# balbasty/torch-interpol

Measured on AMD Instinct MI355X. Metric: Mvox/s grid_pull & grid_push, 256^3 fp32 cubic/dct2, higher is better.
Workload: dtype f32

## Files before the change

### include/interpol_hip.h

```cpp
#ifndef INTERPOL_HIP_H
#define INTERPOL_HIP_H

#include <stdint.h>

#ifdef __cplusplus
extern "C" {
#endif

#define INTERPOL_ABI_VERSION 1

enum {
    INTERPOL_F32  = 0,
    INTERPOL_F64  = 1,
    INTERPOL_BF16 = 2,
    INTERPOL_F16  = 3
};

enum {
    INTERPOL_OK          =  0,
    INTERPOL_E_DIM       = -1,
    INTERPOL_E_ORDER     = -2,
    INTERPOL_E_BOUND     = -3,
    INTERPOL_E_DTYPE     = -4,
    INTERPOL_E_SHAPE     = -5,
    INTERPOL_E_NULL      = -6,
    INTERPOL_E_EXTRAP    = -7,
    INTERPOL_E_PREFILTER = -8,
    INTERPOL_E_SCRATCH   = -9,
    INTERPOL_E_STRIDE    = -10,
    INTERPOL_E_LAUNCH    = -11
};

typedef struct interpol_problem {
    int32_t abi_version;
    int32_t dim;
    int32_t dtype;
    int32_t grid_dtype;
    int32_t extrapolate;
    int32_t bound[3];
    int32_t order[3];
    int32_t flags;
    int64_t batch;
    int64_t channels;
    int64_t vol_shape[3];
    int64_t grid_shape[3];
    int64_t vol_stride[5];
    int64_t grid_stride[5];
    int64_t val_stride[7];
} interpol_problem;

#define INTERPOL_FLAG_NO_FASTPATH   1
#define INTERPOL_FLAG_ACCUMULATE    2
#define INTERPOL_FLAG_FORCE_TILED   4
#define INTERPOL_FLAG_SEPARABLE_GRID 8
#define INTERPOL_FLAG_DISPLACEMENT  16
#define INTERPOL_FLAG_WITH_COUNT    32
#define INTERPOL_FLAG_BINNED_SCATTER 64
#define INTERPOL_FLAG_AUTO_SCATTER  (1 << 24)
#define INTERPOL_FLAG_SMALL_TILES (1 << 25)
#define INTERPOL_FLAG_SERIAL_ITEMS (1 << 26)
#define INTERPOL_FLAG_GENERAL_KERNELS (1 << 27)
#define INTERPOL_FLAG_SHELL_RUNS (1 << 28)
#define INTERPOL_FLAG_AFFINE_GRID   128

int64_t interpol_scatter_workspace(const interpol_problem *p, int32_t count_only);
int interpol_pull(const interpol_problem *p, const void *vol, const void *grid, void *val, void *stream);
int64_t interpol_pull_workspace(const interpol_problem *p);
int interpol_pull_ws(const interpol_problem *p, const void *vol, const void *grid, void *val, void *workspace, int64_t workspace_bytes, void *stream);
int interpol_grad_ws(const interpol_problem *p, const void *vol, const void *grid, void *val, void *workspace, int64_t workspace_bytes, void *stream);
int interpol_push(const interpol_problem *p, const void *val, const void *grid, void *vol,
                  void *scratch, int64_t scratch_bytes, void *stream);
int interpol_count(const interpol_problem *p, const void *grid, void *vol,
                   void *scratch, int64_t scratch_bytes, void *stream);
int interpol_grad(const interpol_problem *p, const void *vol, const void *grid, void *val, void *stream);
int interpol_pushgrad(const interpol_problem *p, const void *val, const void *grid, void *vol,
                      void *scratch, int64_t scratch_bytes, void *stream);
int interpol_hess(const interpol_problem *p, const void *vol, const void *grid, void *val, void *stream);

int interpol_pull_backward(const interpol_problem *p, const void *grad_out, const void *vol, const void *grid,
                           void *grad_vol, void *grad_grid, void *scratch, int64_t scratch_bytes, void *stream);
int interpol_push_backward(const interpol_problem *p, const void *grad_vol_out, const void *val, const void *grid,
                           void *grad_val, void *grad_grid, void *stream);
int interpol_count_backward(const interpol_problem *p, const void *grad_vol_out, const void *grid,
                            void *grad_grid, void *stream);
int interpol_push_backward_ws(const interpol_problem *p, const void *grad_vol_out, const void *val, const void *grid,
                              void *grad_val, void *grad_grid, void *workspace, int64_t workspace_bytes, void *stream);

int64_t interpol_affine_backward_workspace(const interpol_problem *p);
int interpol_pull_backward_affine(const interpol_problem *p, const void *grad_out, const void *vol,
                                  const void *mat, void *grad_mat,
                                  void *workspace, int64_t workspace_bytes, void *stream);
int interpol_push_backward_affine(const interpol_problem *p, const void *grad_vol_out,
                                  const void *val , const void *mat, void *grad_mat,
                                  void *workspace, int64_t workspace_bytes, void *stream);

int interpol_compose(const interpol_problem *p, const void *left, const void *right, void *out, void *stream);
int interpol_compose_backward_right(const interpol_problem *p, const void *grad_out, const void *left, const void *right,
                                    void *grad_right, void *stream);

int interpol_jacobian(const interpol_problem *p, const void *disp, void *out, int det_only, int add_identity, void *stream);
int interpol_jacdet_backward_field(const interpol_problem *p, const void *grad_out, const void *disp, void *gfield, void *stream);

int interpol_regulariser(const interpol_problem *p, const void *field, void *out, double absolute, double membrane, double bending,
                         const double *voxel_size, void *stream);
int64_t interpol_regulariser_energy_workspace(const interpol_problem *p);
int interpol_regulariser_energy(const interpol_problem *p, const void *field, void *energy, double absolute, double membrane,
                                double bending, const double *voxel_size, void *workspace, int64_t workspace_bytes, void *stream);

int64_t interpol_regulariser_solve_workspace(const interpol_problem *p, int hessian_components);
int interpol_regulariser_solve(const interpol_problem *p, const void *gradient, const void *hessian, int hessian_components,
                               int64_t hessian_batch_stride, void *solution, double absolute, double membrane, double bending,
                               const double *voxel_size, int max_iter, double tolerance, void *info ,
                               void *workspace, int64_t workspace_bytes, void *stream);

int64_t interpol_ssd_workspace(const interpol_problem *p);
int interpol_ssd(const interpol_problem *p, const void *moving, const void *fixed, const void *disp, const void *weight ,
                 void *loss, void *gradient, void *hessian, int hessian_kind, int64_t weight_batch_stride,
                 int64_t gradient_batch_stride, int64_t hessian_batch_stride, void *workspace, int64_t workspace_bytes, void *stream);

int64_t interpol_ssd_affine_workspace(const interpol_problem *p);
int interpol_ssd_affine(const interpol_problem *p, const void *moving, const void *fixed, const void *mat, const void *weight ,
                        void *loss, void *gradient, void *hessian, int with_hessian, int64_t mat_batch_stride,
                        int64_t weight_batch_stride, void *workspace, int64_t workspace_bytes, void *stream);

int64_t interpol_mi_affine_workspace(const interpol_problem *p, int bins);
int interpol_mi_affine(const interpol_problem *p, const void *moving, const void *fixed, const void *mat, const void *weight ,
                       const void *ranges, void *loss, void *gradient, void *hessian, void *histogram , int with_hessian,
                       int bins, int64_t mat_batch_stride, int64_t weight_batch_stride, void *workspace, int64_t workspace_bytes,
                       void *stream);

int64_t interpol_lcc_workspace(const interpol_problem *p);
int interpol_lcc(const interpol_problem *p, const void *moving, const void *fixed, const void *disp, const void *weight ,
                 void *loss, void *gradient, void *hessian, int hessian_kind, const int *window, double eps,
                 int64_t weight_batch_stride, int64_t gradient_batch_stride, int64_t hessian_batch_stride, void *workspace,
                 int64_t workspace_bytes, void *stream);

int64_t interpol_push_bricks_workspace(const interpol_problem *p);
int interpol_push_bricks(const interpol_problem *p, const void *val, const void *grid, void *vol,
                         void *workspace, int64_t workspace_bytes, void *stream);

int interpol_pull_labels(const interpol_problem *p, const void *vol, const void *grid, void *val, void *stream);

int interpol_resample_1d(int32_t dtype, int32_t lin_dtype, int32_t order, int32_t bound, int32_t extrapolate, int32_t mode,
                         int32_t adjoint, int64_t outer, int64_t n_samples, int64_t n_lattice, int64_t inner,
                         const void *src, const void *lin, void *dst, void *stream);
int32_t interpol_resample_1d_gathers(int32_t dtype, int64_t n_samples, int64_t inner);

int interpol_spline_filter(void *data, int32_t dtype, int64_t outer, int64_t n, int64_t inner,
                           int32_t bound, int32_t order, void *stream);
int interpol_spline_filter_to(const void *src, void *data, int32_t dtype, int64_t outer, int64_t n, int64_t inner,
                              int32_t bound, int32_t order, void *stream);

int32_t interpol_host_bound_index(int32_t bound, int32_t i, int32_t n);
int32_t interpol_host_bound_sign(int32_t bound, int32_t i, int32_t n);
double  interpol_host_weight(int32_t order, double x, int32_t which);
float   interpol_host_weight_f32(int32_t order, float x, int32_t which);

#define INTERPOL_HANDBACK_ADAPTIVE 0
#define INTERPOL_HANDBACK_ALWAYS   1
#define INTERPOL_HANDBACK_NEVER    2
int32_t interpol_set_handback(int32_t mode);
int32_t interpol_release_stream(void *stream);

int32_t     interpol_abi_version(void);
int32_t     interpol_has_experiments(void);
const char *interpol_error_string(int code);
const char *interpol_kernel_name(const interpol_problem *p, const char *op);

#ifdef __cplusplus
}
#endif
#endif
```

### torch-interpol_amd/csrc/push_owner.hip

```cpp
#include "sorted_util.hpp"
#include "route.hpp"

namespace ip {
namespace owner {

using namespace sorted;

constexpr int BR = 16;
constexpr int OFF = 160;
constexpr int BOX = BR + 3;
constexpr int PZ = BOX;
constexpr int PLANE = BOX * PZ;
constexpr int BOXSLOTS = BOX * PLANE;
constexpr int NCELL = BR * BR * BR;
constexpr int CAPD = 128;
constexpr int CAPX = 512;
constexpr int NT = 512;
constexpr int NS = TS * TS * TS;
constexpr int NT1 = 512, VPT1 = NS / NT1;
constexpr int LB = 6, NBIN = LB * LB * LB;
constexpr int HDR_SHELL = 34;
constexpr int THIN_SHELL_RUN = 16;
constexpr int KMIX = 13;
template <int K> constexpr int KSV = K == KMIX ? 3 : K;
template <int K> __device__ __forceinline__ int kd(const KParams &p, int d) { return K == KMIX ? p.order[d] : K; }
#ifdef IP_OWNER_MIX_TU
#define IP_KS KSV<K>
#define IP_KD(d) kd<K>(p, d)
#define IP_WX(i) own_weight_x<K>(p, tx, i)
#define IP_MU magic_units_p<K>(p)
#else
#define IP_KS K
#define IP_KD(d) K
#define IP_WX(i) weight_x<K>(tx, i)
#define IP_MU magic_units<K>()
#endif

constexpr int NLO = OFF / BR, NHI = (OFF + 3 + BR - 1) / BR;
struct BrickGrid {
    int nb[3];
    int lo[3], top[3], nin[3], split[3];
    int per_item;
    int item;
    int capd;
};
__host__ __device__ __forceinline__ bool folds(int bound, int n) { return (bound == B_REPLICATE || bound == B_DCT1 || bound == B_DCT2) && n >= 2 * BR; }
static BrickGrid brick_grid(const KParams &k)
{
    BrickGrid g;
    const bool mixed = k.order[0] != k.order[1] || k.order[0] != k.order[2];
    for (int d = 0; d < 3; ++d) {
        const int K = mixed ? 3 : k.order[d], n = k.vol_n[d];
        const bool f = folds(k.bound[d], n);
        g.lo[d] = f ? -(BOX - 1) / 2 : 0;
        g.top[d] = f ? n - (BOX + 1) / 2 + BR : (n - K > 0 ? n - K : 0);
        g.nin[d] = (g.top[d] - g.lo[d] + BR - 1) / BR;
        if (f) {
            const int c = g.top[d] - g.lo[d] - BR * (g.nin[d] - 1);
            if (c < K) { g.top[d] -= c; g.nin[d] -= 1; }
        }
        g.split[d] = f ? g.nin[d] / 2 : (g.nin[d] > 0 ? g.nin[d] - 1 : 0);
        g.nb[d] = NLO + g.nin[d] + NHI;
    }
    g.per_item = g.nb[0] * g.nb[1] * g.nb[2];
    g.item = g.per_item; g.capd = 128;
    return g;
}
__host__ __device__ __forceinline__ int brick_and_cell(int ft, int lo, int top, int nin, int split)
{
    if (ft < lo) return ((ft - lo + OFF) >> 4) | (((ft - lo + OFF) & (BR - 1)) << 16);
    if (ft >= top) return (NLO + nin + ((ft - top) >> 4)) | (((ft - top) & (BR - 1)) << 16);
    const int u = ft - lo, v = top - 1 - ft;
    const bool hi = u >= BR * split && (v >> 4) < nin - 1 - split;
    return hi ? (NLO + nin - 1 - (v >> 4)) | ((BR - 1 - (v & (BR - 1))) << 16) : (NLO + (u >> 4)) | ((u & (BR - 1)) << 16);
}
__host__ __device__ __forceinline__ int brick_origin(int bk, int lo, int top, int nin, int split)
{
    if (bk < NLO) return lo + bk * BR - OFF;
    if (bk >= NLO + nin) return top + (bk - NLO - nin) * BR;
    const int j = bk - NLO;
    return j <= split ? lo + j * BR : top - (nin - j) * BR;
}

__device__ __forceinline__ bool shell_brick(const KParams &p, const BrickGrid &bg, int b0, int b1, int b2)
{
    const int bc[3] = { b0, b1, b2 };
    bool shell = false;
#pragma unroll
    for (int d = 0; d < 3; ++d) shell = shell || bc[d] < NLO + (p.bound[d] == B_DST1 ? 1 : 0) || bc[d] >= NLO + bg.nin[d];
    return shell;
}

struct BinSmem {
    int lo[3], total;
    int cnt[NBIN];
    int base[NBIN];
    int bmx[2];
    int orph, pad_;
    int gbk[NBIN];
};

template <typename T>
__device__ __forceinline__ float src_value(const KParams &p, const T *__restrict__ val, int64_t b, int64_t o, int ch, float m)
{
    if (val == nullptr || ch >= p.C) return m;
    return m * Cvt<float, T>::ld(val[b * p.val_sb + ch * p.val_sc + o]);
}

template <typename T, int K, int GM>
__device__ __forceinline__ void scatter_direct(const KParams &p, const T *__restrict__ val, const float *__restrict__ grid, float *__restrict__ vol,
                                            int64_t b, TileGeom g, int tid, unsigned mask, int nch)
{
    Lattice L;
#pragma unroll
    for (int d = 0; d < 3; ++d) { L.bound[d] = p.bound[d]; L.n[d] = p.vol_n[d]; L.ss[d] = p.vol_ss[d] / 4; L.k[d] = kd<K>(p, d); }
    L.lin = 0;
#pragma unroll 1
    for (int v = 0; v < VPT1; ++v) {
        if (!((mask >> v) & 1)) continue;
        int ox, oy, oz; float x[3];
        sample_pos(g, tid + NT1 * v, ox, oy, oz);
        load_xyz<GM>(p, grid, b, g, ox, oy, oz, x);
        const int64_t o = ((int64_t)ox * g.gy + oy) * g.gz + oz;
        const float m = inb_mask(p, x);
        if (KSV<K> == 1 && p.mode == MODE_ISO0) {
            const long long pk0 = wrap_outofline(L.bound[0], __float2int_rn(rintf(x[0])), L.n[0]);
            const long long pk1 = wrap_outofline(L.bound[1], __float2int_rn(rintf(x[1])), L.n[1]);
            const long long pk2 = wrap_outofline(L.bound[2], __float2int_rn(rintf(x[2])), L.n[2]);
            const float sgn = (float)((int)(pk0 >> 32) * (int)(pk1 >> 32) * (int)(pk2 >> 32));
            float *q = vol + b * p.vol_sb + (int)(pk0 & 0xffffffffll) * L.ss[0] + (int)(pk1 & 0xffffffffll) * L.ss[1] + (int)(pk2 & 0xffffffffll) * L.ss[2];
#pragma unroll 1
            for (int ch = 0; ch < nch; ++ch)
                __hip_atomic_fetch_add(q + (int64_t)ch * p.vol_sc, src_value<T>(p, val, b, o, ch, m) * sgn, __ATOMIC_RELAXED, __HIP_MEMORY_SCOPE_AGENT);
            continue;
        }
        int ii[3]; float tt[3];
#pragma unroll
        for (int d = 0; d < 3; ++d) split(kd<K>(p, d), x[d], ii[d], tt[d]);
#pragma unroll 1
        for (int ch = 0; ch < nch; ++ch)
            tiled::scatter_one_thread(L, vol + b * p.vol_sb + ch * p.vol_sc, src_value<T>(p, val, b, o, ch, m), ii[0], ii[1], ii[2], tt[0], tt[1], tt[2]);
    }
}

template <typename T, int K, int GM>
__device__ __forceinline__ void scatter_orphans(const KParams &p, const T *__restrict__ val, const float *__restrict__ grid, float *__restrict__ vol,
                                             int64_t b, TileGeom g, int tid, unsigned mask, int nch)
{
    Lattice L;
#pragma unroll
    for (int d = 0; d < 3; ++d) { L.bound[d] = p.bound[d]; L.n[d] = p.vol_n[d]; L.ss[d] = p.vol_ss[d] / 4; L.k[d] = kd<K>(p, d); }
    L.lin = 0;
#pragma unroll 1
    for (int v = 0; v < VPT1; ++v) {
        unsigned long long todo = __ballot((mask >> v) & 1);
#pragma unroll 1
        while (todo) {
            const int lane = __ffsll((long long)todo) - 1;
            todo &= todo - 1;
            int ox, oy, oz; float x[3];
            sample_pos(g, (tid & ~63) + lane + NT1 * v, ox, oy, oz);
            load_xyz<GM>(p, grid, b, g, ox, oy, oz, x);
            const int64_t o = ((int64_t)ox * g.gy + oy) * g.gz + oz;
            const float m = inb_mask(p, x);
            if (KSV<K> == 1 && p.mode == MODE_ISO0) { x[0] = rintf(x[0]); x[1] = rintf(x[1]); x[2] = rintf(x[2]); }
            int off;
            const float w = tiled::tap_weight_t<-1, -1>(L, x[0], x[1], x[2], tid & 63, &off, nullptr);
            float *q = vol + b * p.vol_sb + off;
#pragma unroll 1
            for (int ch = 0; ch < nch && w != 0.f; ++ch)
                __hip_atomic_fetch_add(q + (int64_t)ch * p.vol_sc, src_value<T>(p, val, b, o, ch, m) * w, __ATOMIC_RELAXED, __HIP_MEMORY_SCOPE_AGENT);
        }
    }
}

template <typename T, int K, int GM>
__device__ __forceinline__ void gather_direct(const KParams &p, const T *__restrict__ img, const float *__restrict__ grid, T *__restrict__ out,
                                              int64_t b, TileGeom g, int tid, unsigned mask)
{
    Lattice L;
#pragma unroll
    for (int d = 0; d < 3; ++d) { L.bound[d] = p.bound[d]; L.n[d] = p.vol_n[d]; L.ss[d] = p.vol_ss[d] / (int)sizeof(T); L.k[d] = kd<K>(p, d); }
    L.lin = 0;
#pragma unroll 1
    for (int v = 0; v < VPT1; ++v) {
        if (!((mask >> v) & 1)) continue;
        int ox, oy, oz; float x[3];
        sample_pos(g, tid + NT1 * v, ox, oy, oz);
        load_xyz<GM>(p, grid, b, g, ox, oy, oz, x);
        const int64_t o = ((int64_t)ox * g.gy + oy) * g.gz + oz;
        const float m = inb_mask(p, x);
        int ii[3]; float tt[3];
#pragma unroll
        for (int d = 0; d < 3; ++d) split(kd<K>(p, d), x[d], ii[d], tt[d]);
#pragma unroll 1
        for (int ch = 0; ch < p.C; ++ch)
            out[b * p.val_sb + ch * p.val_sc + o] = Cvt<float, T>::st(m * tiled::gather_one_thread<T>(L, img + b * p.vol_sb + ch * p.vol_sc, ii[0], ii[1], ii[2], tt[0], tt[1], tt[2], -1));
    }
}

template <typename T, int K, int GM>
__device__ __forceinline__ void gradc_direct(const KParams &p, const T *__restrict__ img, const T *__restrict__ gout, const float *__restrict__ grid,
                                             float *__restrict__ ggrid, int64_t b, TileGeom g, int tid, unsigned mask)
{
    Lattice L;
#pragma unroll
    for (int d = 0; d < 3; ++d) { L.bound[d] = p.bound[d]; L.n[d] = p.vol_n[d]; L.ss[d] = p.vol_ss[d] / (int)sizeof(T); L.k[d] = kd<K>(p, d); }
    L.lin = 0;
#pragma unroll 1
    for (int v = 0; v < VPT1; ++v) {
        if (!((mask >> v) & 1)) continue;
        int ox, oy, oz; float x[3];
        sample_pos(g, tid + NT1 * v, ox, oy, oz);
        load_xyz<GM>(p, grid, b, g, ox, oy, oz, x);
        const int64_t o = ((int64_t)ox * g.gy + oy) * g.gz + oz;
        const float m = inb_mask(p, x);
        int ii[3]; float tt[3];
#pragma unroll
        for (int d = 0; d < 3; ++d) split(kd<K>(p, d), x[d], ii[d], tt[d]);
        float a[3] = { 0.f, 0.f, 0.f };
#pragma unroll 1
        for (int ch = 0; ch < p.C; ++ch) {
            const float gv = gout ? Cvt<float, T>::ld(gout[b * p.val_sb + ch * p.val_sc + o]) : 1.f;
#pragma unroll 1
            for (int d = 0; d < 3; ++d)
                a[d] = __builtin_fmaf(gv, tiled::gather_one_thread<T>(L, img + b * p.vol_sb + ch * p.vol_sc, ii[0], ii[1], ii[2], tt[0], tt[1], tt[2], d), a[d]);
        }
        float *dst = ggrid + (b * p.N + o) * 3;
        dst[0] = a[0] * m; dst[1] = a[1] * m; dst[2] = a[2] * m;
    }
}

template <typename T, int K, int GM>
__device__ __forceinline__ void grad_direct(const KParams &p, const T *__restrict__ img, const float *__restrict__ grid, T *__restrict__ out,
                                            int64_t b, TileGeom g, int tid, unsigned mask)
{
    Lattice L;
#pragma unroll
    for (int d = 0; d < 3; ++d) { L.bound[d] = p.bound[d]; L.n[d] = p.vol_n[d]; L.ss[d] = p.vol_ss[d] / (int)sizeof(T); L.k[d] = kd<K>(p, d); }
    L.lin = 0;
#pragma unroll 1
    for (int v = 0; v < VPT1; ++v) {
        if (!((mask >> v) & 1)) continue;
        int ox, oy, oz; float x[3];
        sample_pos(g, tid + NT1 * v, ox, oy, oz);
        load_xyz<GM>(p, grid, b, g, ox, oy, oz, x);
        const int64_t o = ((int64_t)ox * g.gy + oy) * g.gz + oz;
        const float m = inb_mask(p, x);
        int ii[3]; float tt[3];
#pragma unroll
        for (int d = 0; d < 3; ++d) split(kd<K>(p, d), x[d], ii[d], tt[d]);
#pragma unroll 1
        for (int ch = 0; ch < p.C; ++ch)
#pragma unroll 1
            for (int d = 0; d < 3; ++d)
                out[b * p.val_sb + ch * p.val_sc + 3 * o + d] =
                    Cvt<float, T>::st(m * tiled::gather_one_thread<T>(L, img + b * p.vol_sb + ch * p.vol_sc, ii[0], ii[1], ii[2], tt[0], tt[1], tt[2], d));
    }
}

template <typename T, int K, int GM, int IDX = 0>
__global__ __launch_bounds__(NT1, 4) void own_bin(KParams p, BrickGrid bg, const T *__restrict__ val, const float *__restrict__ grid,
                                               float *__restrict__ vol, int *__restrict__ ndesc, uint2 *__restrict__ desc,
                                               float4 *__restrict__ rec, float *__restrict__ vals, unsigned short *__restrict__ meta,
                                               int *__restrict__ bmax, int64_t nrec,
                                               int gx, int gy, int gz, int nty, int ntz, int ntiles, const int *__restrict__ gate,
                                               const T *__restrict__ aux, const int *__restrict__ all, int blk0, int thin)
{
    const int blk = (int)blockIdx.x + blk0;
    if (IDX) { const bool every = all && *all == 1; if (gate ? (gate[blk] == 0 && !every) : (all && !every)) return; }
    else if (gate && *gate != 1) return;
    extern __shared__ __attribute__((aligned(16))) unsigned char smem_raw[];
    BinSmem &sm = *reinterpret_cast<BinSmem *>(smem_raw);
    const int tid = threadIdx.x;
    const int64_t b = blk / ntiles;
    const TileGeom g = tile_geom(blk % ntiles, gx, gy, gz, nty, ntz);
    const int nch = (IDX || val == nullptr) ? 1 : p.C + p.cc;
    for (int i = tid; i < NBIN; i += NT1) { sm.cnt[i] = 0; sm.gbk[i] = -1; }
    if (tid < 2) sm.bmx[tid] = 0;
    if (tid == 2) sm.orph = 0;
    if (tid < 3) sm.lo[tid] = 0x7fffffff;
    float c[VPT1][3], v0[VPT1], v1[VPT1];
    unsigned valid = 0;
    prof_mark(-1);
    const bool has0 = !IDX && val != nullptr && p.C > 0, has1 = !IDX && val != nullptr && p.C > 1;
    const T *vp0 = has0 ? val + b * p.val_sb : reinterpret_cast<const T *>(grid);
    const T *vp1 = has1 ? val + b * p.val_sb + p.val_sc : reinterpret_cast<const T *>(grid);
#pragma unroll
    for (int v = 0; v < VPT1; ++v) {
        int ox, oy, oz;
        sample_pos(g, tid + NT1 * v, ox, oy, oz);
        if (ox < gx && oy < gy && oz < gz) valid |= 1u << v;
        ox = ox < gx ? ox : gx - 1; oy = oy < gy ? oy : gy - 1; oz = oz < gz ? oz : gz - 1;
        load_xyz<GM>(p, grid, b, g, ox, oy, oz, c[v]);
        const int64_t o = ((int64_t)ox * gy + oy) * gz + oz;
        if (IDX) { v0[v] = __int_as_float((int)o); v1[v] = 0.f; continue; }
        v0[v] = Cvt<float, T>::ld(vp0[has0 ? o : 0]);
        v1[v] = Cvt<float, T>::ld(vp1[has1 ? o : 0]);
    }
    unsigned inbits = 0;
#pragma unroll
    for (int v = 0; v < VPT1 && !IDX; ++v) {
        const float m = inb_mask(p, c[v]);
        v0[v] = has0 ? v0[v] * m : m; v1[v] = has1 ? v1[v] * m : m;
        if (KSV<K> == 1 && m != 0.f) inbits |= 1u << v;
    }
    if (KSV<K> == 1 && !IDX && p.mode == MODE_ISO0) {
#pragma unroll
        for (int v = 0; v < VPT1; ++v) { c[v][0] = rintf(c[v][0]); c[v][1] = rintf(c[v][1]); c[v][2] = rintf(c[v][2]); }
    }
    int bx[VPT1][3];
    unsigned ok = 0;
    int mn[3] = { 0x7fffffff, 0x7fffffff, 0x7fffffff };
#pragma unroll
    for (int v = 0; v < VPT1; ++v) {
        bool in = (valid >> v) & 1;
#pragma unroll
        for (int d = 0; d < 3; ++d) {
            const float fl = floorf(c[v][d] - 0.5f * (float)(kd<K>(p, d) - 1));
            in = in && fl >= (float)(bg.lo[d] - OFF) && fl < (float)(bg.top[d] + NHI * BR);
            bx[v][d] = in ? brick_and_cell(__float2int_rz(fl), bg.lo[d], bg.top[d], bg.nin[d], bg.split[d]) : 0;
        }
        if (in) {
            ok |= 1u << v;
#pragma unroll
            for (int d = 0; d < 3; ++d) mn[d] = (bx[v][d] & 0xffff) < mn[d] ? (bx[v][d] & 0xffff) : mn[d];
        }
    }
    __syncthreads();
    prof_mark(0);
#pragma unroll
    for (int d = 0; d < 3; ++d) {
        const int a = wave_min(mn[d]);
        if ((tid & 63) == 0) atomicMin(&sm.lo[d], a);
    }
    __syncthreads();
    const int lo[3] = { sm.lo[0], sm.lo[1], sm.lo[2] };
    int lbin[VPT1];
    unsigned local = 0;
#pragma unroll
    for (int v = 0; v < VPT1; ++v) {
        const int r0 = (bx[v][0] & 0xffff) - lo[0], r1 = (bx[v][1] & 0xffff) - lo[1], r2 = (bx[v][2] & 0xffff) - lo[2];
        const bool l = ((ok >> v) & 1) && (unsigned)r0 < (unsigned)LB && (unsigned)r1 < (unsigned)LB && (unsigned)r2 < (unsigned)LB;
        lbin[v] = l ? ((r0 * LB + r1) * LB + r2) | ((bx[v][0] >> 16) << 16 | (bx[v][1] >> 16) << 12 | (bx[v][2] >> 16) << 8) : 0;
        if (l) { local |= 1u << v; lbin[v] |= atomicAdd(&sm.cnt[lbin[v] & 255], 1) << 20; }
    }
    __syncthreads();
    prof_mark(1);
    const int64_t tilebase = (int64_t)blk * NS;
    constexpr int PER = (NBIN + 63) / 64;
    int slot[PER];
    if (tid < 64) {
        int cn[PER], s = 0;
#pragma unroll
        for (int i = 0; i < PER; ++i) { const int e = tid * PER + i; cn[i] = e < NBIN ? sm.cnt[e] : 0; s += cn[i]; }
        int incl = s;
#pragma unroll
        for (int o = 1; o < 64; o <<= 1) { const int t = __shfl_up(incl, o); if (tid >= o) incl += t; }
        int run = incl - s;
        if (tid == 63) sm.total = incl;
        unsigned shl = 0;
        int nsh = 0;
        if (!IDX && thin != 0) {
#pragma unroll
            for (int i = 0; i < PER; ++i) {
                const int e = tid * PER + i;
                if (e < NBIN && cn[i] > 0 && shell_brick(p, bg, lo[0] + e / (LB * LB), lo[1] + (e / LB) % LB, lo[2] + e % LB)) { shl |= 1u << i; nsh += cn[i]; }
            }
#pragma unroll
            for (int o = 32; o > 0; o >>= 1) nsh += __shfl_xor(nsh, o);
        }
        const int lim = thin < 0 ? -thin : thin;
#pragma unroll
        for (int i = 0; i < PER; ++i) {
            const int e = tid * PER + i;
            const int r0 = e / (LB * LB), r1 = (e / LB) % LB, r2 = e % LB;
            const int bk = (int)b * bg.item + ((lo[0] + r0) * bg.nb[1] + (lo[1] + r1)) * bg.nb[2] + (lo[2] + r2);
            slot[i] = 0;
            if (e < NBIN) sm.base[e] = run;
            if (e < NBIN && cn[i] > 0) slot[i] = (((shl >> i) & 1) && (thin > 0 ? nsh : cn[i]) <= lim) ? 0x7fffffff : atomicAdd(&ndesc[bk], 1);
            run += cn[i];
        }
    }
    __syncthreads();
    prof_mark(2);
    int pos[VPT1];
#pragma unroll
    for (int v = 0; v < VPT1; ++v)
        pos[v] = ((local >> v) & 1) ? (sm.base[lbin[v] & 255] + (int)((unsigned)lbin[v] >> 20)) | (((lbin[v] >> 8) & 0xfff) << 16) : -1;
    const bool two = nch > 1;
    int amx0 = 0, amx1 = 0;
#pragma unroll
    for (int v = 0; v < VPT1; ++v) {
        if (pos[v] < 0) continue;
        const int64_t at = tilebase + (pos[v] & 0xffff);
        rec[at] = make_float4(c[v][0], c[v][1], c[v][2], v0[v]);
        if (IDX) continue;
        meta[at] = (unsigned short)(pos[v] >> 16);
        const int a0 = __float_as_int(__builtin_fabsf(v0[v]));
        amx0 = a0 > amx0 ? a0 : amx0;
        if (two) {
            vals[at] = v1[v];
            const int a1 = __float_as_int(__builtin_fabsf(v1[v]));
            amx1 = a1 > amx1 ? a1 : amx1;
        }
    }
    for (int ch = 2; ch < nch && !IDX; ++ch) {
#pragma unroll
        for (int v = 0; v < VPT1; ++v) {
            if (pos[v] < 0) continue;
            int ox, oy, oz;
            sample_pos(g, tid + NT1 * v, ox, oy, oz);
            vals[(int64_t)(ch - 1) * nrec + tilebase + (pos[v] & 0xffff)] = src_value<T>(p, val, b, ((int64_t)ox * gy + oy) * gz + oz, ch, KSV<K> == 1 ? (float)((inbits >> v) & 1u) : inb_mask(p, c[v]));
        }
    }
    if (tid < 64) {
#pragma unroll
        for (int i = 0; i < PER; ++i) {
            const int e = tid * PER + i;
            const int cn = e < NBIN ? sm.cnt[e] : 0;
            if (cn <= 0) continue;
            const int r0 = e / (LB * LB), r1 = (e / LB) % LB, r2 = e % LB;
            const int bk = (int)b * bg.item + ((lo[0] + r0) * bg.nb[1] + (lo[1] + r1)) * bg.nb[2] + (lo[2] + r2);
            if (slot[i] < bg.capd) {
                desc[(int64_t)bk * bg.capd + slot[i]] = make_uint2((unsigned)(tilebase + sm.base[e]), (unsigned)cn);
                sm.gbk[e] = bk;
                if (!IDX && shell_brick(p, bg, lo[0] + r0, lo[1] + r1, lo[2] + r2)) ndesc[HDR_SHELL - 64] = 1;
                if (IDX && slot[i] == 0) bmax[1 + atomicAdd(&bmax[0], 1)] = bk;
            } else { sm.cnt[e] = -1; sm.orph = 1; }
        }
    }
    if (!IDX) {
        amx0 = wave_max(amx0); amx1 = wave_max(amx1);
        if ((tid & 63) == 0) { if (amx0) atomicMax(&sm.bmx[0], amx0); if (amx1) atomicMax(&sm.bmx[1], amx1); }
    }
    __syncthreads();
    for (int e = tid; e < NBIN && !IDX; e += NT1) {
        const int bk = sm.gbk[e];
        if (bk < 0) continue;
        if (sm.bmx[0]) atomicMax(&bmax[2 * (int64_t)bk], sm.bmx[0]);
        if (sm.bmx[1]) atomicMax(&bmax[2 * (int64_t)bk + 1], sm.bmx[1]);
    }
    unsigned direct = valid & ~local;
    if (sm.orph) {
        unsigned orphan = 0;
#pragma unroll
        for (int v = 0; v < VPT1; ++v)
            if (((local >> v) & 1) && sm.cnt[lbin[v] & 255] < 0) orphan |= 1u << v;
        if (IDX) direct |= orphan;
        else scatter_orphans<T, K, GM>(p, val, grid, vol, b, g, tid, orphan, nch);
    }
    if (IDX == 3) { if (direct) grad_direct<T, K, GM>(p, val, grid, reinterpret_cast<T *>(vol), b, g, tid, direct); return; }
    if (IDX == 2) { if (direct) gradc_direct<T, K, GM>(p, val, aux, grid, vol, b, g, tid, direct); return; }
    if (IDX) { if (direct) gather_direct<T, K, GM>(p, val, grid, reinterpret_cast<T *>(vol), b, g, tid, direct); return; }
    if (direct) scatter_direct<T, K, GM>(p, val, grid, vol, b, g, tid, direct, nch);
}

constexpr int VPT = 12;
constexpr int NPIECE = VPT * (NT / 64);
constexpr int BATCH = NPIECE * 64;
constexpr int NCLS = 16;
constexpr int NHW = NT / NCLS;
constexpr unsigned PMASK = 0x1ffffffu;
static_assert(NPIECE <= 128, "a queue entry is piece << 6 | lane in 16 bits");

struct AccSmem {
    int   taboff[3][BOX + 1];
    float tabsgn[3][BOX + 1];
    unsigned ppref[CAPX];
    unsigned start[CAPX];
    uint2 piece[NPIECE];
    int   cmax[2];
    int   dmax, n, npieces;
    int   rlo[3], rhi[3];
    int   qcnt[NCLS];
    int   qsur[NCLS + 1], qhol[NCLS + 1];
    int   qeff[NCLS], qcap;
    union alignas(16) {
        struct {
            unsigned cells[NCELL / 2];
            unsigned short queue[BATCH];
        };
        unsigned nreg[BOX * BOX * (BOX + 1) / 2];
    };
    unsigned long long box[BOXSLOTS];
};
constexpr int NZ = BOX + 1;
static_assert(sizeof(AccSmem) <= 80 * 1024, "two workgroups per CU");
static_assert(sizeof(unsigned) * (BOX * BOX * NZ / 2) <= sizeof(unsigned) * (NCELL / 2) + sizeof(unsigned short) * BATCH, "the stencil counts fit in cells + queue");

constexpr float MAGIC = 12582912.f;
constexpr unsigned MAGIC_ODD = 301u;
template <int K> __device__ __forceinline__ float magic_units() { return K == 3 ? 4194304.f * 0.999f * 3.375f : (K == 2 ? 4194304.f * 0.999f * (64.f / 27.f) : 4194304.f * 0.999f); }
template <int K> __device__ __forceinline__ float magic_cbmax() { return 2147483648.f * 0.99f / magic_units<K>(); }
template <int K> __device__ __forceinline__ float magic_units_p(const KParams &p)
{
    if (K != KMIX) return magic_units<K>();
    float u = 4194304.f * 0.999f;
#pragma unroll
    for (int d = 0; d < 3; ++d) u *= p.order[d] == 3 ? 1.5f : (p.order[d] == 2 ? 4.f / 3.f : 1.f);
    return u;
}

__device__ __forceinline__ void magic_decode(unsigned long long W, unsigned n, int &s0, int &s1)
{
    const unsigned pr = n * MAGIC_ODD;
    const unsigned mlo = pr << 22, mhi = pr >> 10;
    s0 = (int)((unsigned)W - mlo);
    const unsigned long long L = (((unsigned long long)mhi << 32) | mlo) + (unsigned long long)(long long)s0;
    s1 = (int)((unsigned)(W >> 32) - mlo - (unsigned)(L >> 32));
}

template <int I, int J, int NZT = 4>
__device__ __forceinline__ void row_adds(unsigned addr, unsigned long long v0, unsigned long long v1, unsigned long long v2, unsigned long long v3)
{
    constexpr int o = (I * PLANE + J * PZ) * 8;
    if (NZT == 4)
        asm volatile("ds_add_u64 %0, %1 offset:%5\n\tds_add_u64 %0, %2 offset:%6\n\tds_add_u64 %0, %3 offset:%7\n\tds_add_u64 %0, %4 offset:%8"
                     :: "v"(addr), "v"(v0), "v"(v1), "v"(v2), "v"(v3), "n"(o), "n"(o + 8), "n"(o + 16), "n"(o + 24) : "memory");
    else if (NZT == 3)
        asm volatile("ds_add_u64 %0, %1 offset:%4\n\tds_add_u64 %0, %2 offset:%5\n\tds_add_u64 %0, %3 offset:%6"
                     :: "v"(addr), "v"(v0), "v"(v1), "v"(v2), "n"(o), "n"(o + 8), "n"(o + 16) : "memory");
    else
        asm volatile("ds_add_u64 %0, %1 offset:%3\n\tds_add_u64 %0, %2 offset:%4"
                     :: "v"(addr), "v"(v0), "v"(v1), "n"(o), "n"(o + 8) : "memory");
}
template <int K, int I, int J, bool WIDE>
__device__ __forceinline__ void scatter_row(unsigned addr, f2 sx, const f2 *w, int dbg)
{
    const f2 sy = sx * f2{ w[J].x, w[J].x };
    unsigned long long v[4];
#pragma unroll
    for (int k = 0; k < 4; ++k) {
        if (WIDE) {
            v[k] = (unsigned long long)(long long)tiled::cvt_rpi(sy.x * w[k].y);
        } else {
            const f2 pr = __builtin_elementwise_fma(sy, f2{ w[k].y, w[k].y }, f2{ MAGIC, MAGIC });
            v[k] = __builtin_bit_cast(unsigned long long, pr);
        }
    }
#ifdef IP_ABLATE
    if (dbg & 4) { asm volatile("" :: "v"(v[0]), "v"(v[1]), "v"(v[2]), "v"(v[3])); return; }
#endif
    row_adds<I, J, WIDE ? 4 : IP_KS + 1>(addr, v[0], v[1], v[2], v[3]);
}
template <int K, int I, bool WIDE>
__device__ __forceinline__ void scatter_plane(unsigned addr, f2 s, float wxi, const f2 *w, int dbg)
{
#ifdef IP_ABLATE
    if (dbg & 16) {
        const unsigned long long c = 0x100000001ull;
        row_adds<I, 0>(addr, c, c, c, c); row_adds<I, 1>(addr, c, c, c, c); row_adds<I, 2>(addr, c, c, c, c);
        if (IP_KS == 3) row_adds<I, 3>(addr, c, c, c, c);
        return;
    }
#endif
    const f2 sx = s * f2{ wxi, wxi };
    scatter_row<K, I, 0, WIDE>(addr, sx, w, dbg); scatter_row<K, I, 1, WIDE>(addr, sx, w, dbg);
    if (IP_KS >= 2) scatter_row<K, I, 2, WIDE>(addr, sx, w, dbg);
    if (IP_KS == 3) scatter_row<K, I, 3, WIDE>(addr, sx, w, dbg);
}

typedef unsigned short us2 __attribute__((ext_vector_type(2)));
template <int W>
__device__ __forceinline__ void slide(const unsigned *in, unsigned *out)
{
    us2 s = { 0, 0 };
#pragma unroll
    for (int j = 0; j < BOX; ++j) {
        if (j < BR) s += __builtin_bit_cast(us2, in[j]);
        if (j >= W && j - W < BR) s -= __builtin_bit_cast(us2, in[j - W]);
        out[j] = __builtin_bit_cast(unsigned, s);
    }
}
template <int K, typename SM>
__device__ __forceinline__ void stencil_counts(SM &sm, int tid)
{
    constexpr int W = IP_KS + 1, HZ = NZ / 2;
    unsigned *rg = sm.nreg;
    unsigned in[BR], out[BOX];
    if (tid < BR * BR) {
        const uint4 lo = reinterpret_cast<const uint4 *>(sm.cells)[2 * tid], hi = reinterpret_cast<const uint4 *>(sm.cells)[2 * tid + 1];
        in[0] = lo.x; in[1] = lo.y; in[2] = lo.z; in[3] = lo.w; in[4] = hi.x; in[5] = hi.y; in[6] = hi.z; in[7] = hi.w;
    }
    __syncthreads();
    if (tid < BR * BR) {
        int v[BR], o[NZ], s = 0;
#pragma unroll
        for (int i = 0; i < BR / 2; ++i) { v[2 * i] = (int)(in[i] & 0xffffu); v[2 * i + 1] = (int)(in[i] >> 16); }
#pragma unroll
        for (int j = 0; j < BOX; ++j) { if (j < BR) s += v[j]; if (j >= W && j - W < BR) s -= v[j - W]; o[j] = s; }
        o[BOX] = 0;
#pragma unroll
        for (int i = 0; i < HZ; ++i) rg[tid * HZ + i] = (unsigned)o[2 * i] | ((unsigned)o[2 * i + 1] << 16);
    }
    __syncthreads();
    {
        const int x = tid / HZ, zp = tid - x * HZ;
        if (tid < BR * HZ) {
#pragma unroll
            for (int k = 0; k < BR; ++k) in[k] = rg[(x * BR + k) * HZ + zp];
        }
        __syncthreads();
        if (tid < BR * HZ) {
            slide<W>(in, out);
#pragma unroll
            for (int j = 0; j < BOX; ++j) rg[(x * BOX + j) * HZ + zp] = out[j];
        }
        __syncthreads();
    }
    {
        const int y = tid / HZ, zp = tid - y * HZ;
        if (tid < BOX * HZ) {
#pragma unroll
            for (int k = 0; k < BR; ++k) in[k] = rg[(k * BOX + y) * HZ + zp];
        }
        __syncthreads();
        if (tid < BOX * HZ) {
            slide<W>(in, out);
#pragma unroll
            for (int j = 0; j < BOX; ++j) rg[(j * BOX + y) * HZ + zp] = out[j];
        }
        __syncthreads();
    }
}
__device__ __forceinline__ unsigned stencils_at(const AccSmem &sm, int xr, int yr, int zr)
{
    return (unsigned)reinterpret_cast<const unsigned short *>(sm.nreg)[(xr * BOX + yr) * NZ + zr];
}

template <int K> __device__ __forceinline__ float own_weight_x(const KParams &p, float t, int i)
{
    if constexpr (K == KMIX) return mixed_weight_x(p.order[0], t, i);
    else return weight_x<K>(t, i);
}
template <int K> __device__ __forceinline__ float own_wgrad_x(const KParams &p, float t, int i)
{
    if constexpr (K == KMIX) return mixed_wgrad_x(p.order[0], t, i);
    else return wgrad_x<K>(t, i);
}
#ifdef IP_OWNER_MIX_TU
#define IP_RECORD_CELL(...) record_cell<K>(p, __VA_ARGS__)
template <int K>
__device__ __forceinline__ void record_cell(const KParams &p, const float4 &r, const int *b0, int &x0, int &y0, int &z0, float &tx, float &ty, float &tz)
{
    const float fx = floorf(r.x - 0.5f * (float)(kd<K>(p, 0) - 1)), fy = floorf(r.y - 0.5f * (float)(kd<K>(p, 1) - 1)), fz = floorf(r.z - 0.5f * (float)(kd<K>(p, 2) - 1));
#else
#define IP_RECORD_CELL(...) record_cell<K>(__VA_ARGS__)
template <int K>
__device__ __forceinline__ void record_cell(const float4 &r, const int *b0, int &x0, int &y0, int &z0, float &tx, float &ty, float &tz)
{
    const float fx = floorf(r.x - 0.5f * (float)(K - 1)), fy = floorf(r.y - 0.5f * (float)(K - 1)), fz = floorf(r.z - 0.5f * (float)(K - 1));
#endif
    tx = r.x - fx; ty = r.y - fy; tz = r.z - fz;
    x0 = (__float2int_rz(fx) - b0[0]) & (BR - 1); y0 = (__float2int_rz(fy) - b0[1]) & (BR - 1); z0 = (__float2int_rz(fz) - b0[2]) & (BR - 1);
}

__host__ __device__ __forceinline__ int color_first(int color, int d)
{
    if (color >= 8) return 0;
    const int par = (color >> (2 - d)) & 1;
    return NLO + ((par - NLO) & 1);
}
__host__ __device__ __forceinline__ int color_count(int color, int d, const BrickGrid &bg)
{
    if (color >= 8) return bg.nb[d];
    const int j0 = color_first(color, d) - NLO;
    return bg.nin[d] > j0 ? (bg.nin[d] - j0 + 1) >> 1 : 0;
}

template <int K, typename SM>
__device__ __forceinline__ void float_records(const Lattice &L, const SM &sm, float *vc0, float *vc1, bool two, const float4 *__restrict__ rec,
                                              const float *__restrict__ va, const float *__restrict__ vb, const int *b0, int ebeg, int eend)
{
#pragma unroll 1
    for (int e = ebeg; e < eend; e += NHW) {
        const unsigned qe = sm.queue[e];
        const unsigned ri = sm.piece[qe >> 6].x + (qe & 63u);
        const float4 cur = rec[ri];
        const float cs[2] = { va ? va[ri] : cur.w, vb ? vb[ri] : 0.f };
        int x0, y0, z0; float tx, ty, tz;
        record_cell<K>(cur, b0, x0, y0, z0, tx, ty, tz);
#pragma unroll 1
        for (int i = 0; i <= K; ++i) {
            const int gx = b0[0] + x0 + i;
            const int offx = wrap_index(L.bound[0], gx, L.n[0]) * L.ss[0];
            const float fx = tiled::weight1(0, K, tx, i), gsx = (float)wrap_sign(L.bound[0], gx, L.n[0]);
            const float sx0 = cs[0] * fx * gsx, sx1 = cs[1] * fx * gsx;
#pragma unroll 1
            for (int j = 0; j <= K; ++j) {
                const int gy = b0[1] + y0 + j;
                const int offy = wrap_index(L.bound[1], gy, L.n[1]) * L.ss[1];
                const float fy = tiled::weight1(0, K, ty, j), gsy = (float)wrap_sign(L.bound[1], gy, L.n[1]);
                const float sy0 = sx0 * fy * gsy, sy1 = sx1 * fy * gsy;
#pragma unroll 1
                for (int k = 0; k <= K; ++k) {
                    const int gz = b0[2] + z0 + k;
                    const int off = offx + offy + wrap_index(L.bound[2], gz, L.n[2]) * L.ss[2];
                    const float fz = tiled::weight1(0, K, tz, k), gsz = (float)wrap_sign(L.bound[2], gz, L.n[2]);
                    __hip_atomic_fetch_add(vc0 + off, sy0 * fz * gsz, __ATOMIC_RELAXED, __HIP_MEMORY_SCOPE_AGENT);
                    if (two) __hip_atomic_fetch_add(vc1 + off, sy1 * fz * gsz, __ATOMIC_RELAXED, __HIP_MEMORY_SCOPE_AGENT);
                }
            }
        }
    }
}

template <int K, bool NEAR = false, bool SHELL = true>
__global__ __launch_bounds__(NT, 4) void own_accumulate(KParams p, BrickGrid bg, const int *__restrict__ ndesc, const uint2 *__restrict__ desc,
                                                        const float4 *__restrict__ rec, const float *__restrict__ vals,
                                                        const unsigned short *__restrict__ meta, const int *__restrict__ bmax, int64_t nrec,
                                                        float *__restrict__ vol, int nch, int color, int nbatch, const int *__restrict__ gate,
                                                        int *__restrict__ ctr, int bfirst, const int *__restrict__ shell)
{
    if (gate && *gate != 1) return;
    static_assert(SHELL || (K != KMIX && !NEAR), "the colour instantiation: isotropic orders 1 - 3");
    if (SHELL) { if (color == 8 && *shell == 0) return; }
    else __builtin_assume(color >= 0 && color < 8);
    extern __shared__ __attribute__((aligned(16))) unsigned char smem_raw[];
    AccSmem &sm = *reinterpret_cast<AccSmem *>(smem_raw);
    Lattice L;
#pragma unroll
    for (int d = 0; d < 3; ++d) { L.bound[d] = p.bound[d]; L.n[d] = p.vol_n[d]; L.ss[d] = p.vol_ss[d] / 4; L.k[d] = IP_KD(d); }
    L.lin = 0;
    const int step = !SHELL || color < 8 ? 2 : 1;
    const int c0[3] = { color_first(color, 0), color_first(color, 1), color_first(color, 2) };
    const int m0 = color_count(color, 0, bg), m1 = color_count(color, 1, bg), m2 = color_count(color, 2, bg);
    const int nwork = m0 * m1 * m2 * nbatch;
    for (int e = threadIdx.x; e < BOXSLOTS; e += NT) sm.box[e] = 0ull;
    const bool dynamic = !SHELL || color < 8;
    __shared__ int next_chunk;
    for (int round = 0; ; ++round) {
    int chunk, stride;
    if (dynamic) {
        __syncthreads();
        if (threadIdx.x == 0) next_chunk = atomicAdd(ctr, 1);
        __syncthreads();
        chunk = next_chunk; stride = nwork;
    } else {
        chunk = (int)blockIdx.x + round * 64 * (int)gridDim.x; stride = (int)gridDim.x;
    }
    if (chunk >= nwork) break;
    unsigned long long pending = 1ull;
    if (SHELL) {
        const long long wl = (long long)chunk + (long long)(threadIdx.x & 63) * stride;
        const int w = wl < nwork ? (int)wl : nwork;
        bool take = false;
        if (w < nwork) {
            int r = w;
            const int iz = r % m2; r /= m2;
            const int iy = r % m1; r /= m1;
            const int ix = r % m0;
            const int bb = r / m0 + bfirst;
            const int bx_[3] = { ix * step + c0[0], iy * step + c0[1], iz * step + c0[2] };
            bool interior = true;
#pragma unroll
            for (int d = 0; d < 3; ++d) interior = interior && bx_[d] >= NLO + (L.bound[d] == B_DST1 ? 1 : 0) && bx_[d] < NLO + bg.nin[d];
            if (color < 8 ? interior : (color == 9 || !interior))
                take = ndesc[bb * bg.item + (bx_[0] * bg.nb[1] + bx_[1]) * bg.nb[2] + bx_[2]] != 0;
        }
        pending = __ballot(take);
    }
    while (pending) {
        const int work = chunk + (__ffsll((long long)pending) - 1) * stride;
        pending &= pending - 1;
        const int tid = opaque((int)threadIdx.x);
        int r = work;
        const int iz = r % m2; r /= m2;
        const int iy = r % m1; r /= m1;
        const int ix = r % m0;
        const int64_t b = r / m0 + bfirst;
        const int bxyz[3] = { ix * step + c0[0], iy * step + c0[1], iz * step + c0[2] };
        const int b0[3] = { brick_origin(bxyz[0], bg.lo[0], bg.top[0], bg.nin[0], bg.split[0]), brick_origin(bxyz[1], bg.lo[1], bg.top[1], bg.nin[1], bg.split[1]),
                            brick_origin(bxyz[2], bg.lo[2], bg.top[2], bg.nin[2], bg.split[2]) };
        bool interior = true;
#pragma unroll
        for (int d = 0; d < 3; ++d) interior = interior && bxyz[d] >= NLO + (L.bound[d] == B_DST1 ? 1 : 0) && bxyz[d] < NLO + bg.nin[d];
        if (!SHELL || color < 8 ? !interior : (color == 8 && interior)) continue;
        const bool atomic = SHELL && color >= 8;
        bool edge = false;
#pragma unroll
        for (int d = 0; d < 3; ++d) edge = edge || b0[d] < 0 || b0[d] + BOX > L.n[d];
        edge = edge && !atomic;
        int foldmul = 1;
        if (edge) {
#pragma unroll
            for (int d = 0; d < 3; ++d) {
                const int nout = b0[d] < 0 ? -b0[d] : (b0[d] + BOX > L.n[d] ? b0[d] + BOX - L.n[d] : 0);
                foldmul *= nout == 0 ? 1 : (L.bound[d] == B_REPLICATE ? nout + 1 : 2);
            }
        }
        const int brick = (int)b * bg.item + (bxyz[0] * bg.nb[1] + bxyz[1]) * bg.nb[2] + bxyz[2];
        int nd = ndesc[brick];
        if (nd == 0) continue;
        nd = nd < bg.capd ? nd : bg.capd;
        __syncthreads();
        prof_mark(-1);
        if (tid < 64) {
            constexpr int PER = CAPX / 64;
            int cn[PER], np[PER], s = 0, sp = 0; unsigned st_[PER];
#pragma unroll
            for (int i = 0; i < PER; ++i) {
                const int e = tid * PER + i;
                const uint2 dsc = e < nd ? desc[(int64_t)brick * bg.capd + e] : make_uint2(0u, 0u);
                cn[i] = (int)dsc.y; st_[i] = dsc.x; np[i] = (cn[i] + 63) >> 6; s += cn[i]; sp += np[i];
            }
            int incl = s, inclp = sp;
#pragma unroll
            for (int o = 1; o < 64; o <<= 1) {
                const int t = __shfl_up(incl, o), tp = __shfl_up(inclp, o);
                if (tid >= o) { incl += t; inclp += tp; }
            }
            int runp = inclp - sp;
#pragma unroll
            for (int i = 0; i < PER; ++i) {
                const int e = tid * PER + i;
                const unsigned last = cn[i] > 0 ? (unsigned)(cn[i] - 64 * (np[i] - 1)) : 0u;
                sm.ppref[e] = e < nd ? ((unsigned)runp & PMASK) | (last << 25) : 0xffffffffu;
                sm.start[e] = st_[i];
                runp += np[i];
            }
            if (tid == 63) { sm.n = incl; sm.npieces = inclp; sm.dmax = 0; sm.cmax[0] = 0; sm.cmax[1] = 0; }
            if (SHELL && tid < 3) { sm.rlo[tid] = BR; sm.rhi[tid] = -1; }
        } else if (atomic && tid < 64 + 3 * 32) {
            const int d = (tid - 64) >> 5, slot = tid & 31;
            if (slot < BOX) {
                const long long pk = wrap_outofline(L.bound[d], b0[d] + slot, L.n[d]);
                sm.taboff[d][slot] = (int)(pk & 0xffffffffll) * L.ss[d];
                sm.tabsgn[d][slot] = (float)(int)(pk >> 32);
            }
        }
        for (int e = tid; e < NCELL / 2; e += NT) sm.cells[e] = 0u;
        if (tid < NCLS) sm.qcnt[tid] = 0;
        __syncthreads();
        const int n = sm.n, npieces = sm.npieces;
        const int wave = tid >> 6, lane = tid & 63;
        auto build_pieces = [&](int pb0) {
            if (tid < NPIECE) {
                const int g = pb0 + tid;
                uint2 pc = make_uint2(0u, 0u);
                if (g < npieces) {
                    int j = 0;
#pragma unroll
                    for (int st = CAPX / 2; st > 0; st >>= 1) j += (int)(sm.ppref[j + st] & PMASK) <= g ? st : 0;
                    const unsigned pj = sm.ppref[j];
                    const int q = g - (int)(pj & PMASK);
                    const int nextp = j + 1 < CAPX ? (int)(sm.ppref[j + 1] & PMASK) : (int)PMASK;
                    const bool lastp = g + 1 == (nextp < npieces ? nextp : npieces);
                    pc = make_uint2(sm.start[j] + 64u * (unsigned)q, lastp ? (pj >> 25) : 64u);
                }
                sm.piece[tid] = pc;
            }
            __syncthreads();
        };
        prof_mark(8);
        if (NEAR) {
            float *boxf = reinterpret_cast<float *>(sm.box);
            for (int c = 0; c < nch; c += 2) {
                const bool two = c + 1 < nch;
                float *vc0 = vol + b * p.vol_sb + c * p.vol_sc;
                float *vc1 = two ? vc0 + p.vol_sc : vc0;
                const float *va = c == 0 ? nullptr : vals + (int64_t)(c - 1) * nrec;
                const float *vb = two ? vals + (int64_t)c * nrec : nullptr;
                for (int pb0 = 0; pb0 < npieces; pb0 += NPIECE) {
                    if (pb0 > 0 || c > 0) __syncthreads();
                    build_pieces(pb0);
#pragma unroll 1
                    for (int k = 0; k < VPT; ++k) {
                        const uint2 pc = sm.piece[wave + k * (NT / 64)];
                        if (lane >= (int)pc.y) continue;
                        const unsigned ri = pc.x + (unsigned)lane;
                        const float4 rc = rec[ri];
                        const float s0 = va ? va[ri] : rc.w, s1 = vb ? vb[ri] : 0.f;
                        int ii[3] = { __float2int_rn(rc.x), __float2int_rn(rc.y), __float2int_rn(rc.z) };
                        float sgn = 1.f;
                        if (atomic || ii[0] < 0 || ii[0] >= L.n[0] || ii[1] < 0 || ii[1] >= L.n[1] || ii[2] < 0 || ii[2] >= L.n[2]) {
#pragma unroll
                            for (int d = 0; d < 3; ++d) {
                                const long long pk = wrap_outofline(L.bound[d], ii[d], L.n[d]);
                                ii[d] = (int)(pk & 0xffffffffll); sgn *= (float)(int)(pk >> 32);
                            }
                        }
                        const int xr = ii[0] - b0[0], yr = ii[1] - b0[1], zr = ii[2] - b0[2];
                        if (atomic || (unsigned)xr >= (unsigned)BOX || (unsigned)yr >= (unsigned)BOX || (unsigned)zr >= (unsigned)BOX) {
                            const int off = ii[0] * L.ss[0] + ii[1] * L.ss[1] + ii[2] * L.ss[2];
                            __hip_atomic_fetch_add(vc0 + off, s0 * sgn, __ATOMIC_RELAXED, __HIP_MEMORY_SCOPE_AGENT);
                            if (two) __hip_atomic_fetch_add(vc1 + off, s1 * sgn, __ATOMIC_RELAXED, __HIP_MEMORY_SCOPE_AGENT);
                            continue;
                        }
                        float *slot = boxf + 2 * (xr * PLANE + yr * PZ + zr);
                        __builtin_amdgcn_ds_faddf((__attribute__((address_space(3))) float *)slot, s0 * sgn, 0, 0, false);
                        if (two) __builtin_amdgcn_ds_faddf((__attribute__((address_space(3))) float *)(slot + 1), s1 * sgn, 0, 0, false);
                    }
                }
                __syncthreads();
                if (!atomic) {
                    constexpr int UF0 = 7;
#pragma unroll 1
                    for (int e0 = tid; e0 < BOXSLOTS; e0 += UF0 * NT) {
                        int off[UF0]; float a0[UF0], a1[UF0], t0[UF0], t1[UF0];
                        unsigned nz = 0;
#pragma unroll
                        for (int u = 0; u < UF0; ++u) {
                            const int e = e0 + u * NT;
                            off[u] = 0; a0[u] = 0.f; a1[u] = 0.f;
                            if (e < BOXSLOTS) {
                                a0[u] = boxf[2 * e]; a1[u] = boxf[2 * e + 1];
                                if (a0[u] != 0.f || a1[u] != 0.f) {
                                    const int xr = e / PLANE, rem = e - xr * PLANE, yr = rem / PZ, zr = rem - yr * PZ;
                                    off[u] = (b0[0] + xr) * L.ss[0] + (b0[1] + yr) * L.ss[1] + (b0[2] + zr) * L.ss[2];
                                    nz |= 1u << u;
                                    sm.box[e] = 0ull;
                                }
                            }
                        }
#pragma unroll
                        for (int u = 0; u < UF0; ++u) {
                            t0[u] = ((nz >> u) & 1) ? vc0[off[u]] : 0.f;
                            t1[u] = (((nz >> u) & 1) && two) ? vc1[off[u]] : 0.f;
                        }
#pragma unroll
                        for (int u = 0; u < UF0; ++u) {
                            if (!((nz >> u) & 1)) continue;
                            vc0[off[u]] = t0[u] + a0[u];
                            if (two) vc1[off[u]] = t1[u] + a1[u];
                        }
                    }
                }
                __syncthreads();
            }
            continue;
        }
        int qr[VPT];
        if (tid == 0) { sm.cmax[0] = bmax[2 * (int64_t)brick]; sm.cmax[1] = nch > 1 ? bmax[2 * (int64_t)brick + 1] : 0; }
        for (int pb0 = 0; pb0 < npieces; pb0 += NPIECE) {
            if (pb0 > 0) __syncthreads();
            build_pieces(pb0);
            unsigned mk[VPT];
#pragma unroll
            for (int k = 0; k < VPT; ++k) {
                const uint2 pc = sm.piece[wave + k * (NT / 64)];
                mk[k] = lane < (int)pc.y ? (unsigned)meta[pc.x + (unsigned)lane] : 0xffffffffu;
            }
#pragma unroll
            for (int k = 0; k < VPT; ++k) {
                if (pb0 == 0) qr[k] = -1;
                if (mk[k] != 0xffffffffu) {
                    const int x0 = (mk[k] >> 8) & 15, y0 = (mk[k] >> 4) & 15, z0 = mk[k] & 15;
                    const int cell = (int)(mk[k] & 4095u);
                    atomicAdd(&sm.cells[cell >> 1], 1u << (16 * (cell & 1)));
                    if (pb0 == 0) {
                        const int q = (x0 * PLANE + y0 * PZ + z0) & (NCLS - 1);
                        qr[k] = q | (atomicAdd(&sm.qcnt[q], 1) << 4);
                    }
                }
            }
        }
        __syncthreads();
        prof_mark(9);
        {
            int dm = 0;
            int mn[3] = { BR, BR, BR }, mx[3] = { -1, -1, -1 };
            for (int e = tid; e < NCELL / 2; e += NT) {
                const unsigned w2 = sm.cells[e];
                const int a = (int)(w2 & 0xffffu), c2 = (int)(w2 >> 16);
                dm = a > dm ? a : dm; dm = c2 > dm ? c2 : dm;
                if (atomic && w2) {
                    const int x0 = e >> 7, y0 = (e >> 3) & 15, z0 = (2 * e) & 15;
                    mn[0] = x0 < mn[0] ? x0 : mn[0]; mx[0] = x0 > mx[0] ? x0 : mx[0];
                    mn[1] = y0 < mn[1] ? y0 : mn[1]; mx[1] = y0 > mx[1] ? y0 : mx[1];
                    mn[2] = z0 < mn[2] ? z0 : mn[2]; mx[2] = z0 + 1 > mx[2] ? z0 + 1 : mx[2];
                }
            }
            dm = wave_max(dm);
            if (lane == 0 && dm > 0) atomicMax(&sm.dmax, dm);
            if (atomic) {
#pragma unroll
                for (int d = 0; d < 3; ++d) {
                    const int a = wave_min(mn[d]), c2 = wave_max(mx[d]);
                    if (lane == 0) { atomicMin(&sm.rlo[d], a); atomicMax(&sm.rhi[d], c2); }
                }
            }
        }
        __syncthreads();
        prof_mark(10);
#ifdef IP_OWNER_MIX_TU
        float wsum3 = 1.f;
#pragma unroll
        for (int d = 0; d < 3; ++d) wsum3 *= kd<K>(p, d) == 3 ? 1.6666667f : (kd<K>(p, d) == 2 ? 1.75f : 2.f);
        const bool dense = n >= 60000 || (float)(sm.dmax * foldmul) * wsum3 > 2147483648.f * 0.99f / magic_units_p<K>(p);
#else
        const float wsum = K == 3 ? 1.6666667f : (K == 2 ? 1.75f : 2.f);
        const bool dense = n >= 60000 || (float)(sm.dmax * foldmul) * (wsum * wsum * wsum) > magic_cbmax<K>();
#endif
        const bool one_batch = npieces <= NPIECE;
        for (int c = 0; c < nch; c += 2) {
            const bool two = c + 1 < nch;
            float *vc0 = vol + b * p.vol_sb + c * p.vol_sc;
            float *vc1 = two ? vc0 + p.vol_sc : vc0;
            const float *va = c == 0 ? nullptr : vals + (int64_t)(c - 1) * nrec;
            const float *vb = two ? vals + (int64_t)c * nrec : nullptr;
            if (c > 0) {
                float am0 = 0.f, am1 = 0.f;
                for (int e = tid; e < NCELL / 2; e += NT) sm.cells[e] = 0u;
                __syncthreads();
                for (int pb0 = 0; pb0 < npieces; pb0 += NPIECE) {
                    if (!one_batch) { __syncthreads(); build_pieces(pb0); }
                    for (int k = 0; k < VPT; ++k) {
                        const uint2 pc = sm.piece[wave + k * (NT / 64)];
                        if (lane >= (int)pc.y) continue;
                        const unsigned ri = pc.x + (unsigned)lane;
                        const int cell = (int)(meta[ri] & 4095u);
                        atomicAdd(&sm.cells[cell >> 1], 1u << (16 * (cell & 1)));
                        const float a0 = __builtin_fabsf(va[ri]), a1 = two ? __builtin_fabsf(vb[ri]) : 0.f;
                        am0 = (a0 > am0 || a0 != a0) ? a0 : am0;
                        am1 = (a1 > am1 || a1 != a1) ? a1 : am1;
                    }
                }
                const int w0 = wave_max(__float_as_int(am0)), w1 = wave_max(__float_as_int(am1));
                if (lane == 0) { if (w0) atomicMax(&sm.cmax[0], w0); if (w1) atomicMax(&sm.cmax[1], w1); }
                __syncthreads();
            }
            const int mb0 = sm.cmax[0], mb1 = sm.cmax[1];
            const bool fin = (mb0 & 0x7f800000) != 0x7f800000 && (mb1 & 0x7f800000) != 0x7f800000;
            const bool wide = dense && fin;
            const bool fixedpt = fin && !(p.dbg & 8);
            int ex0 = ((mb0 >> 23) & 0xff) - 127, ex1 = ((mb1 >> 23) & 0xff) - 127;
            ex0 = ex0 < -90 ? -90 : ex0; ex1 = ex1 < -90 ? -90 : ex1;
            const float a0 = fmaxf(__int_as_float(mb0), 1e-27f), a1 = fmaxf(__int_as_float(mb1), 1e-27f);
            const f2 scale = { mb0 ? IP_MU / a0 : 0.f, mb1 ? IP_MU / a1 : 0.f };
            const float inv0 = a0 * (1.f / IP_MU), inv1 = a1 * (1.f / IP_MU);
            const f2 scalew = { mb0 ? __int_as_float((127 + 30 - ex0) << 23) : 0.f, mb1 ? __int_as_float((127 + 30 - ex1) << 23) : 0.f };
            const float invw0 = __int_as_float((127 - 30 + ex0) << 23), invw1 = __int_as_float((127 - 30 + ex1) << 23);
            const unsigned boxaddr = (unsigned)(size_t)(__attribute__((address_space(3))) void *)(sm.box);
            for (int sub = 0; sub < (wide && two ? 2 : 1); ++sub) {
            for (int pb0 = 0; pb0 < npieces; pb0 += NPIECE) {
                const int tid = opaque((int)threadIdx.x);
                const int wave = tid >> 6, lane = tid & 63;
                if (pb0 > 0 || c > 0 || sub > 0) {
                    __syncthreads();
                    if (tid < NCLS) sm.qcnt[tid] = 0;
                    if (!one_batch) build_pieces(pb0); else __syncthreads();
#pragma unroll
                    for (int k = 0; k < VPT; ++k) {
                        const uint2 pc = sm.piece[wave + k * (NT / 64)];
                        qr[k] = -1;
                        if (lane < (int)pc.y) {
                            const unsigned mk = meta[pc.x + (unsigned)lane];
                            const int x0 = (mk >> 8) & 15, y0 = (mk >> 4) & 15, z0 = mk & 15;
                            const int q = (x0 * PLANE + y0 * PZ + z0) & (NCLS - 1);
                            qr[k] = q | (atomicAdd(&sm.qcnt[q], 1) << 4);
                        }
                    }
                    __syncthreads();
                } else if (!one_batch) {
                    __syncthreads();
                    build_pieces(0);
                }
                if (tid < 32) {
                    const bool cls = tid < NCLS;
                    const int cq = cls ? sm.qcnt[tid] : 0;
                    int tot, nsur, nhol;
                    half_excl_scan(cq, tot);
                    const int cap = (((tot + NCLS - 1) / NCLS) + NHW - 1) / NHW * NHW;
                    const int sur = cls && cq > cap ? cq - cap : 0, hol = cls && cq < cap ? cap - cq : 0;
                    const int so = half_excl_scan(sur, nsur), ho = half_excl_scan(hol, nhol);
                    if (cls) { sm.qsur[tid] = so; sm.qhol[tid] = ho; }
                    if (tid == 31) { sm.qsur[NCLS] = nsur; sm.qhol[NCLS] = nhol; sm.qcap = cap; }
                    const int fill = nsur - ho < 0 ? 0 : (nsur - ho > hol ? hol : nsur - ho);
                    if (cls) sm.qeff[tid] = (cq < cap ? cq : cap) + fill;
                }
                __syncthreads();
                const int qcap = sm.qcap;
#pragma unroll
                for (int k = 0; k < VPT; ++k) {
                    if (qr[k] < 0) continue;
                    const int qq = qr[k] & (NCLS - 1), r = qr[k] >> 4;
                    int slot = qq * qcap + r;
                    if (r >= qcap) {
                        const int o = sm.qsur[qq] + r - qcap;
                        int c2 = 0;
#pragma unroll
                        for (int st = NCLS / 2; st > 0; st >>= 1) if (sm.qhol[c2 + st] <= o) c2 += st;
                        slot = c2 * qcap + sm.qcnt[c2] + (o - sm.qhol[c2]);
                    }
                    sm.queue[slot] = (unsigned short)(((wave + k * (NT / 64)) << 6) | lane);
                }
                __syncthreads();
                const int q = tid & (NCLS - 1), hw = tid >> 4;
                const int ebeg = q * qcap + hw, eend = q * qcap + sm.qeff[q];
                const int nit = qcap / NHW;
                auto fetch = [&](int e, float4 &rc, float &s0, float &s1) {
                    const unsigned qe = sm.queue[e];
                    const unsigned ri = sm.piece[qe >> 6].x + (qe & 63u);
                    rc = rec[ri]; s0 = va ? va[ri] : rc.w; s1 = vb ? vb[ri] : 0.f;
                };
                if constexpr (!SHELL) {
                    auto taps = [&](auto widec) {
                        constexpr bool WIDE = decltype(widec)::value;
                        float4 rc = make_float4(0.f, 0.f, 0.f, 0.f); float s0 = 0.f, s1 = 0.f;
                        if (ebeg < eend) fetch(ebeg, rc, s0, s1);
#pragma unroll 1
                        for (int it = 0; it < nit; ++it) {
                            const int e = ebeg + it * NHW;
                            const float4 cur = rc; const float cs0 = s0, cs1 = s1;
                            if (e + NHW < eend) fetch(e + NHW, rc, s0, s1);
                            if (e >= eend) continue;
                            int x0, y0, z0; float tx, ty, tz;
                            IP_RECORD_CELL(cur, b0, x0, y0, z0, tx, ty, tz);
#ifdef IP_ABLATE
                            if (p.dbg & 2) continue;
#endif
                            unsigned addr = boxaddr + 8u * (unsigned)(x0 * PLANE + y0 * PZ + z0);
                            f2 w[4];
                            weights_yz<K>(f2{ ty, tz }, w);
                            const f2 ss = WIDE ? (sub ? f2{ cs1 * scalew.y, 0.f } : f2{ cs0 * scalew.x, 0.f }) : f2{ cs0, cs1 } * scale;
                            scatter_plane<K, 0, WIDE>(addr, ss, IP_WX(0), w, p.dbg);
                            scatter_plane<K, 1, WIDE>(addr, ss, IP_WX(1), w, p.dbg);
                            if (IP_KS >= 2) scatter_plane<K, 2, WIDE>(addr, ss, IP_WX(2), w, p.dbg);
                            if (IP_KS == 3) scatter_plane<K, 3, WIDE>(addr, ss, IP_WX(3), w, p.dbg);
                        }
                    };
                    if (!fixedpt) float_records<K>(L, sm, vc0, vc1, two, rec, va, vb, b0, ebeg, eend);
                    else if (wide) taps(std::true_type{});
                    else taps(std::false_type{});
                } else {
                    float4 rc = make_float4(0.f, 0.f, 0.f, 0.f); float s0 = 0.f, s1 = 0.f;
                    if (ebeg < eend) fetch(ebeg, rc, s0, s1);
#pragma unroll 1
                    for (int it = 0; it < nit; ++it) {
                        const int e = ebeg + it * NHW;
                        const float4 cur = rc; const float cs0 = s0, cs1 = s1;
                        if (e + NHW < eend) fetch(e + NHW, rc, s0, s1);
                        if (e >= eend) continue;
                        int x0, y0, z0; float tx, ty, tz;
                        IP_RECORD_CELL(cur, b0, x0, y0, z0, tx, ty, tz);
                        if (fixedpt) {
#ifdef IP_ABLATE
                            if (p.dbg & 2) continue;
#endif
                            unsigned addr = boxaddr + 8u * (unsigned)(x0 * PLANE + y0 * PZ + z0);
                            f2 w[4];
#ifdef IP_OWNER_MIX_TU
                            if constexpr (K == KMIX) mixed_weights_yz(p.order[1], p.order[2], f2{ ty, tz }, w);
                            else
#endif
                            weights_yz<K>(f2{ ty, tz }, w);
                            if (wide) {
                                const f2 ss = sub ? f2{ cs1 * scalew.y, 0.f } : f2{ cs0 * scalew.x, 0.f };
                                scatter_plane<K, 0, true>(addr, ss, IP_WX(0), w, p.dbg);
                                scatter_plane<K, 1, true>(addr, ss, IP_WX(1), w, p.dbg);
                                if (IP_KS >= 2) scatter_plane<K, 2, true>(addr, ss, IP_WX(2), w, p.dbg);
                                if (IP_KS == 3) scatter_plane<K, 3, true>(addr, ss, IP_WX(3), w, p.dbg);
                            } else {
                                const f2 ss = f2{ cs0, cs1 } * scale;
                                scatter_plane<K, 0, false>(addr, ss, IP_WX(0), w, p.dbg);
                                scatter_plane<K, 1, false>(addr, ss, IP_WX(1), w, p.dbg);
                                if (IP_KS >= 2) scatter_plane<K, 2, false>(addr, ss, IP_WX(2), w, p.dbg);
                                if (IP_KS == 3) scatter_plane<K, 3, false>(addr, ss, IP_WX(3), w, p.dbg);
                            }
                        } else {
                            tiled::scatter_one_thread(L, vc0, cs0, b0[0] + x0, b0[1] + y0, b0[2] + z0, tx, ty, tz);
                            if (two) tiled::scatter_one_thread(L, vc1, cs1, b0[0] + x0, b0[1] + y0, b0[2] + z0, tx, ty, tz);
                        }
                    }
                }
            }
            asm volatile("s_waitcnt lgkmcnt(0)" ::: "memory");
            __syncthreads();
            prof_mark(11);
            const bool magic = fixedpt && !wide;
            if (magic) stencil_counts<K>(sm, tid);
            prof_mark(13);
            if (edge && fixedpt) {
#pragma unroll
                for (int d = 0; d < 3; ++d) {
                    const int nlo = b0[d] < 0 ? -b0[d] : 0, nhi = b0[d] + BOX > L.n[d] ? b0[d] + BOX - L.n[d] : 0;
                    if (nlo + nhi == 0) continue;
                    for (int i = tid; i < (nlo + nhi) * (BOX * BOX); i += NT) {
                        const int o = i / (BOX * BOX), rest = i - o * (BOX * BOX), r1 = rest / BOX, r2 = rest - r1 * BOX;
                        const int rd = o < nlo ? o : BOX - nhi + (o - nlo);
                        const int idx = b0[d] + rd;
                        int j;
                        if (L.bound[d] == B_REPLICATE) j = idx < 0 ? 0 : L.n[d] - 1;
                        else if (L.bound[d] == B_DCT1) j = idx < 0 ? -idx : 2 * L.n[d] - 2 - idx;
                        else j = idx < 0 ? -1 - idx : 2 * L.n[d] - 1 - idx;
                        const int rt = j - b0[d];
                        const int es = d == 0 ? rd * PLANE + r1 * PZ + r2 : d == 1 ? r1 * PLANE + rd * PZ + r2 : r1 * PLANE + r2 * PZ + rd;
                        const int et = d == 0 ? rt * PLANE + r1 * PZ + r2 : d == 1 ? r1 * PLANE + rt * PZ + r2 : r1 * PLANE + r2 * PZ + rt;
                        const unsigned long long v = sm.box[es];
                        if (v) { sm.box[es] = 0ull; atomicAdd(&sm.box[et], v); }
                        if (magic) {
                            const int ns = d == 0 ? (rd * BOX + r1) * NZ + r2 : d == 1 ? (r1 * BOX + rd) * NZ + r2 : (r1 * BOX + r2) * NZ + rd;
                            const int nt = d == 0 ? (rt * BOX + r1) * NZ + r2 : d == 1 ? (r1 * BOX + rt) * NZ + r2 : (r1 * BOX + r2) * NZ + rt;
                            unsigned short *nn = reinterpret_cast<unsigned short *>(sm.nreg);
                            const unsigned c2 = nn[ns];
                            if (c2) { nn[ns] = 0; atomicAdd(&sm.nreg[nt >> 1], c2 << (16 * (nt & 1))); }
                        }
                    }
                    __syncthreads();
                }
            }
            if (fixedpt && !atomic && !wide && !(p.dbg & 1)) {
                constexpr int UF2 = 7;
#pragma unroll 1
                for (int e0 = tid; e0 < BOXSLOTS; e0 += UF2 * NT) {
                    int off[UF2]; float t0[UF2], t1[UF2];
                    unsigned nz = 0, nst[UF2];
#pragma unroll
                    for (int u = 0; u < UF2; ++u) {
                        const int e = e0 + u * NT;
                        off[u] = 0;
                        if (e < BOXSLOTS) {
                            const int xr = e / PLANE, rem = e - xr * PLANE, yr = rem / PZ, zr = rem - yr * PZ;
                            off[u] = (b0[0] + xr) * L.ss[0] + (b0[1] + yr) * L.ss[1] + (b0[2] + zr) * L.ss[2];
                            nst[u] = stencils_at(sm, xr, yr, zr);
                            if (nst[u] != 0u) nz |= 1u << u;
                        }
                    }
#pragma unroll
                    for (int u = 0; u < UF2; ++u) {
                        t0[u] = ((nz >> u) & 1) ? vc0[off[u]] : 0.f;
                        t1[u] = (((nz >> u) & 1) && two) ? vc1[off[u]] : 0.f;
                    }
#pragma unroll
                    for (int u = 0; u < UF2; ++u) {
                        if (!((nz >> u) & 1)) continue;
                        const int e = e0 + u * NT;
                        const unsigned long long a = sm.box[e];
                        sm.box[e] = 0ull;
                        int lo_, hi_;
                        magic_decode(a, nst[u], lo_, hi_);
                        vc0[off[u]] = t0[u] + (float)lo_ * inv0;
                        if (two) vc1[off[u]] = t1[u] + (float)hi_ * inv1;
                    }
                }
            } else if (fixedpt && !(p.dbg & 1)) {
                constexpr int UF = 4;
                const int fl0 = atomic ? sm.rlo[0] : 0, fl1 = atomic ? sm.rlo[1] : 0, fl2 = atomic ? sm.rlo[2] : 0;
                const int fe1 = atomic ? sm.rhi[1] + IP_KS - fl1 + 1 : BOX, fe2 = atomic ? sm.rhi[2] + IP_KS - fl2 + 1 : BOX;
                const int nflush = atomic ? (sm.rhi[0] + IP_KS - fl0 + 1) * fe1 * fe2 : BOXSLOTS;
                const float r2 = 1.f / (float)fe2, r1 = 1.f / (float)fe1;
                for (int e0 = tid; e0 < nflush; e0 += UF * NT) {
                    long long a[UF]; int off[UF]; float sg[UF]; unsigned nst[UF];
#pragma unroll
                    for (int u = 0; u < UF; ++u) {
                        int e = e0 + u * NT;
                        a[u] = 0; off[u] = 0; sg[u] = 1.f; nst[u] = 0u;
                        if (e < nflush) {
                            int xr, yr, zr;
                            if (atomic) {
                                const int t = (int)(((float)e + 0.5f) * r2);
                                zr = e - t * fe2 + fl2;
                                xr = (int)(((float)t + 0.5f) * r1);
                                yr = t - xr * fe1 + fl1; xr += fl0;
                                e = xr * PLANE + yr * PZ + zr;
                            } else {
                                xr = e / PLANE; const int rem = e - xr * PLANE; yr = rem / PZ; zr = rem - yr * PZ;
                            }
                            a[u] = (long long)sm.box[e];
                            sm.box[e] = 0ull;
                            if (!wide) nst[u] = stencils_at(sm, xr, yr, zr);
                            if (atomic) {
                                off[u] = sm.taboff[0][xr] + sm.taboff[1][yr] + sm.taboff[2][zr];
                                sg[u] = sm.tabsgn[0][xr] * sm.tabsgn[1][yr] * sm.tabsgn[2][zr];
                            } else {
                                off[u] = (b0[0] + xr) * L.ss[0] + (b0[1] + yr) * L.ss[1] + (b0[2] + zr) * L.ss[2];
                            }
                        }
                    }
                    if (wide) {
                        float *vcs = sub ? vc1 : vc0;
                        const float invs = sub ? invw1 : invw0;
#pragma unroll
                        for (int u = 0; u < UF; ++u) {
                            if (a[u] == 0) continue;
                            const float val = (float)((double)a[u] * (double)(invs * sg[u]));
                            if (atomic) __hip_atomic_fetch_add(vcs + off[u], val, __ATOMIC_RELAXED, __HIP_MEMORY_SCOPE_AGENT);
                            else vcs[off[u]] += val;
                        }
                    } else if (atomic) {
#pragma unroll
                        for (int u = 0; u < UF; ++u) {
                            if (nst[u] == 0u) continue;
                            int lo_, hi_;
                            magic_decode((unsigned long long)a[u], nst[u], lo_, hi_);
                            if (lo_ != 0) __hip_atomic_fetch_add(vc0 + off[u], (float)lo_ * (inv0 * sg[u]), __ATOMIC_RELAXED, __HIP_MEMORY_SCOPE_AGENT);
                            if (hi_ != 0 && two) __hip_atomic_fetch_add(vc1 + off[u], (float)hi_ * (inv1 * sg[u]), __ATOMIC_RELAXED, __HIP_MEMORY_SCOPE_AGENT);
                        }
                    } else {
                        float t0[UF], t1[UF];
#pragma unroll
                        for (int u = 0; u < UF; ++u) {
                            t0[u] = nst[u] != 0u ? vc0[off[u]] : 0.f;
                            t1[u] = (nst[u] != 0u && two) ? vc1[off[u]] : 0.f;
                        }
#pragma unroll
                        for (int u = 0; u < UF; ++u) {
                            if (nst[u] == 0u) continue;
                            int lo_, hi_;
                            magic_decode((unsigned long long)a[u], nst[u], lo_, hi_);
                            vc0[off[u]] = t0[u] + (float)lo_ * inv0;
                            if (two) vc1[off[u]] = t1[u] + (float)hi_ * inv1;
                        }
                    }
                }
            }
            __syncthreads();
            }
            prof_mark(12);
            if (tid == 0) { sm.cmax[0] = 0; sm.cmax[1] = 0; }
        }
    }
    }
}

static __global__ void own_zero(int *__restrict__ p, int n)
{
    const int i = blockIdx.x * 1024 + threadIdx.x;
    if (i < n) p[i] = 0;
}


constexpr int GPZ = 20;
constexpr int GPLANE = BOX * GPZ;
struct GatSmem {
    int   taboff[3][BOX + 1];
    float tabsgn[3][BOX + 1];
    unsigned start[CAPD];
    int   pref[CAPD + 2];
    int   brick, pad;
    float2 box[BOX * GPLANE];
};
#define IP_RD(o, off) "ds_read_b64 %" #o ", %16 offset:" #off "\n\t"
__device__ __forceinline__ void gather_reads(unsigned addr, f2 (&v)[16])
{
    static_assert(GPZ * 8 == 160, "the immediate offsets are (row * GPZ + k) * 8");
    asm volatile(IP_RD(0, 0) IP_RD(1, 8) IP_RD(2, 16) IP_RD(3, 24)
                 IP_RD(4, 160) IP_RD(5, 168) IP_RD(6, 176) IP_RD(7, 184)
                 IP_RD(8, 320) IP_RD(9, 328) IP_RD(10, 336) IP_RD(11, 344)
                 IP_RD(12, 480) IP_RD(13, 488) IP_RD(14, 496) IP_RD(15, 504)
                 "s_waitcnt lgkmcnt(0)"
                 : "=&v"(v[0]), "=&v"(v[1]), "=&v"(v[2]), "=&v"(v[3]), "=&v"(v[4]), "=&v"(v[5]), "=&v"(v[6]), "=&v"(v[7]),
                   "=&v"(v[8]), "=&v"(v[9]), "=&v"(v[10]), "=&v"(v[11]), "=&v"(v[12]), "=&v"(v[13]), "=&v"(v[14]), "=&v"(v[15])
                 : "v"(addr) : "memory");
}
#undef IP_RD

template <int K, int GRAD = 0>
__global__ __launch_bounds__(NT, 4) void own_gather(KParams p, BrickGrid bg, const int *__restrict__ ndesc, const uint2 *__restrict__ desc,
                                                    const float4 *__restrict__ rec, const int *__restrict__ list, int *__restrict__ draw,
                                                    const float *__restrict__ img, float *__restrict__ out, const int *__restrict__ gate,
                                                    const float *__restrict__ gout)
{
    if (gate && *gate != 1) return;
    extern __shared__ __attribute__((aligned(16))) unsigned char smem_raw[];
    GatSmem &sm = *reinterpret_cast<GatSmem *>(smem_raw);
    const int nlist = list[0];
    for (;;) {
        const int tid = opaque((int)threadIdx.x);
        __syncthreads();
        if (tid == 0) { const int i = atomicAdd(draw, 1); sm.brick = i < nlist ? list[1 + i] : -1; }
        __syncthreads();
        const int bk = sm.brick;
        if (bk < 0) break;
        const int64_t b = bk / bg.per_item;
        int r = bk - (int)b * bg.per_item;
        const int bz = r % bg.nb[2]; r /= bg.nb[2];
        const int by = r % bg.nb[1], bx = r / bg.nb[1];
        const int b0[3] = { brick_origin(bx, bg.lo[0], bg.top[0], bg.nin[0], bg.split[0]), brick_origin(by, bg.lo[1], bg.top[1], bg.nin[1], bg.split[1]),
                            brick_origin(bz, bg.lo[2], bg.top[2], bg.nin[2], bg.split[2]) };
        const int nd = min(ndesc[bk], CAPD);
        if (tid >= 256 && tid < 320) {
            static_assert(CAPD == 128, "two runs per lane");
            const int ln = tid - 256, e0 = 2 * ln, e1 = e0 + 1;
            const uint2 d0 = e0 < nd ? desc[(int64_t)bk * CAPD + e0] : make_uint2(0u, 0u), d1 = e1 < nd ? desc[(int64_t)bk * CAPD + e1] : make_uint2(0u, 0u);
            const int sum = (int)d0.y + (int)d1.y;
            int incl = sum;
#pragma unroll
            for (int o = 1; o < 64; o <<= 1) { const int t = __shfl_up(incl, o); if (ln >= o) incl += t; }
            sm.start[e0] = d0.x; sm.start[e1] = d1.x;
            sm.pref[e0] = incl - sum; sm.pref[e1] = incl - (int)d1.y;
            if (ln == 63) { sm.pref[CAPD] = incl; sm.pref[CAPD + 1] = 0x7fffffff; }
        }
        if (tid < 3 * 64) {
            const int d = tid >> 6, slot = tid & 63;
            if (slot < BOX) {
                const long long pk = wrap_outofline(p.bound[d], (d == 0 ? b0[0] : d == 1 ? b0[1] : b0[2]) + slot, p.vol_n[d]);
                sm.taboff[d][slot] = (int)(pk & 0xffffffffll) * (p.vol_ss[d] / 4);
                sm.tabsgn[d][slot] = (float)(int)(pk >> 32);
            }
        }
        for (int c = 0; c < p.C; c += 2) {
            const bool two = c + 1 < p.C;
            const float *vc0 = img + b * p.vol_sb + (int64_t)c * p.vol_sc;
            const float *vc1 = two ? vc0 + p.vol_sc : vc0;
            float *oc0 = out + b * p.val_sb + (int64_t)c * p.val_sc;
            __syncthreads();
            const bool zlin = p.vol_ss[2] == 4 && b0[2] >= (p.bound[2] == B_DST1 ? 1 : 0) && b0[2] + BOX <= p.vol_n[2];
            if (p.dbg & 1) {
            } else if (zlin) {
                for (int e = tid; e < BOX * BOX * 5; e += NT) {
                    const int row = e / 5, q = e - row * 5;
                    const int x = row / BOX, y = row - x * BOX;
                    const int zs = q < 4 ? 4 * q : BOX - 4;
                    const int off = sm.taboff[0][x] + sm.taboff[1][y] + b0[2] + zs;
                    const float sg = sm.tabsgn[0][x] * sm.tabsgn[1][y];
                    const float4 a0 = ld4<float>(vc0 + off), a1 = ld4<float>(vc1 + off);
                    float2 *dst = sm.box + row * GPZ + zs;
                    if (q < 4) {
                        reinterpret_cast<float4 *>(dst)[0] = make_float4(a0.x * sg, a1.x * sg, a0.y * sg, a1.y * sg);
                        reinterpret_cast<float4 *>(dst)[1] = make_float4(a0.z * sg, a1.z * sg, a0.w * sg, a1.w * sg);
                    } else {
                        dst[0] = make_float2(a0.x * sg, a1.x * sg); dst[1] = make_float2(a0.y * sg, a1.y * sg);
                        dst[2] = make_float2(a0.z * sg, a1.z * sg); dst[3] = make_float2(a0.w * sg, a1.w * sg);
                    }
                }
            } else {
                for (int e = tid; e < BOX * BOX * BOX; e += NT) {
                    const int x = e / (BOX * BOX), y = (e / BOX) % BOX, z = e % BOX;
                    const int off = sm.taboff[0][x] + sm.taboff[1][y] + sm.taboff[2][z];
                    const float sg = sm.tabsgn[0][x] * sm.tabsgn[1][y] * sm.tabsgn[2][z];
                    sm.box[(x * BOX + y) * GPZ + z] = make_float2(vc0[off] * sg, vc1[off] * sg);
                }
            }
            __syncthreads();
            const unsigned boxaddr = (unsigned)(size_t)(__attribute__((address_space(3))) void *)(sm.box);
            const int ntot = sm.pref[CAPD];
            int rr = 0;
            for (int j = tid; j < ntot; j += NT) {
                {
                    while (j >= sm.pref[rr + 1]) ++rr;
                    const float4 rc = rec[sm.start[rr] + (unsigned)(j - sm.pref[rr])];
                    const float fx = floorf(rc.x - 0.5f * (float)(kd<K>(p, 0) - 1)), fy = floorf(rc.y - 0.5f * (float)(kd<K>(p, 1) - 1)), fz = floorf(rc.z - 0.5f * (float)(kd<K>(p, 2) - 1));
                    const float tx = rc.x - fx; const f2 tyz = f2{ rc.y - fy, rc.z - fz };
                    int cx = __float2int_rz(fx) - b0[0], cy = __float2int_rz(fy) - b0[1], cz = __float2int_rz(fz) - b0[2];
                    cx = max(0, min(cx, BR - 1)); cy = max(0, min(cy, BR - 1)); cz = max(0, min(cz, BR - 1));
                    const unsigned addr = boxaddr + (unsigned)((cx * BOX + cy) * GPZ + cz) * 8u;
                    float wx[4];
                    {
                        if constexpr (K == KMIX) weights4(p.order[0], tx, wx);
                        else if (K == 3) { const float u = tx - 1.f, v = 2.f - tx, u2 = u * u, v2 = v * v;
                                      wx[0] = (v2 * v) * (1.f / 6.f); wx[3] = (u2 * u) * (1.f / 6.f); wx[1] = u2 * (u * 0.5f - 1.f) + 2.f / 3.f; wx[2] = v2 * (v * 0.5f - 1.f) + 2.f / 3.f; }
                        else { const float a = 1.5f - tx, cc = tx - 0.5f, m = tx - 1.f; wx[0] = (a * a) * 0.5f; wx[1] = 0.75f - m * m; wx[2] = (cc * cc) * 0.5f; wx[3] = 0.f; }
                    }
                    f2 w[4];
                    if constexpr (K == KMIX) mixed_weights_yz(p.order[1], p.order[2], tyz, w);
                    else weights_yz<K>(tyz, w);
                    if (GRAD == 2) {
                        f2 dq[4];
                        if constexpr (K == KMIX) mixed_wgrads_yz(p.order[1], p.order[2], tyz, dq);
                        else wgrads_yz<K>(tyz, dq);
                        f2 g0 = { 0.f, 0.f }, g1 = { 0.f, 0.f }, g2 = { 0.f, 0.f };
#pragma unroll
                        for (int ii = 0; ii <= KSV<K>; ++ii) {
                            if (K == KMIX && ii > p.order[0]) continue;
                            f2 t2[16];
                            gather_reads(addr + (unsigned)(ii * GPLANE * 8), t2);
                            if constexpr (K == KMIX) clear_unused_taps(p.order[1], p.order[2], t2);
                            f2 pp = { 0.f, 0.f }, ppy = { 0.f, 0.f }, ppz = { 0.f, 0.f };
#pragma unroll
                            for (int jy = 0; jy <= KSV<K>; ++jy) {
                                f2 q = { 0.f, 0.f }, qz = { 0.f, 0.f };
#pragma unroll
                                for (int k = 0; k <= KSV<K>; ++k) {
                                    q = f2{ w[k].y, w[k].y } * t2[4 * jy + k] + q;
                                    qz = f2{ dq[k].y, dq[k].y } * t2[4 * jy + k] + qz;
                                }
                                pp = f2{ w[jy].x, w[jy].x } * q + pp;
                                ppy = f2{ dq[jy].x, dq[jy].x } * q + ppy;
                                ppz = f2{ w[jy].x, w[jy].x } * qz + ppz;
                            }
                            const float wxi = own_weight_x<K>(p, tx, ii), gxi = own_wgrad_x<K>(p, tx, ii);
                            g0 = f2{ gxi, gxi } * pp + g0;
                            g1 = f2{ wxi, wxi } * ppy + g1;
                            g2 = f2{ wxi, wxi } * ppz + g2;
                            asm volatile("" : "+v"(g0), "+v"(g1), "+v"(g2));
                        }
                        const float xyz[3] = { rc.x, rc.y, rc.z };
                        const float m = inb_mask(p, xyz);
                        float *dst = oc0 + 3 * (int64_t)__float_as_int(rc.w);
                        dst[0] = g0.x * m; dst[1] = g1.x * m; dst[2] = g2.x * m;
                        if (two) { dst[p.val_sc] = g0.y * m; dst[p.val_sc + 1] = g1.y * m; dst[p.val_sc + 2] = g2.y * m; }
                        continue;
                    }
                    if (GRAD == 1) {
                        const int64_t o = (int64_t)__float_as_int(rc.w);
                        const float *gc0 = gout ? gout + b * p.val_sb + (int64_t)c * p.val_sc : nullptr;
                        const float go0 = gc0 ? gc0[o] : 1.f, go1 = two ? (gc0 ? gc0[p.val_sc + o] : 1.f) : 0.f;
                        f2 dq[4];
                        if constexpr (K == KMIX) mixed_wgrads_yz(p.order[1], p.order[2], tyz, dq);
                        else wgrads_yz<K>(tyz, dq);
                        float ag0 = 0.f, ag1 = 0.f, ag2 = 0.f;
#pragma unroll
                        for (int ii = 0; ii <= KSV<K>; ++ii) {
                            if (K == KMIX && ii > p.order[0]) continue;
                            f2 t2[16];
                            gather_reads(addr + (unsigned)(ii * GPLANE * 8), t2);
                            if constexpr (K == KMIX) clear_unused_taps(p.order[1], p.order[2], t2);
                            float pp = 0.f, ppy = 0.f, ppz = 0.f;
#pragma unroll
                            for (int jy = 0; jy <= KSV<K>; ++jy) {
                                float q = 0.f, qz = 0.f;
#pragma unroll
                                for (int k = 0; k <= KSV<K>; ++k) {
                                    const float sgl = __builtin_fmaf(go1, t2[4 * jy + k].y, go0 * t2[4 * jy + k].x);
                                    q = __builtin_fmaf(w[k].y, sgl, q);
                                    qz = __builtin_fmaf(dq[k].y, sgl, qz);
                                }
                                pp = __builtin_fmaf(w[jy].x, q, pp);
                                ppy = __builtin_fmaf(dq[jy].x, q, ppy);
                                ppz = __builtin_fmaf(w[jy].x, qz, ppz);
                            }
                            const float wxi = own_weight_x<K>(p, tx, ii);
                            ag0 = __builtin_fmaf(own_wgrad_x<K>(p, tx, ii), pp, ag0);
                            ag1 = __builtin_fmaf(wxi, ppy, ag1);
                            ag2 = __builtin_fmaf(wxi, ppz, ag2);
                            asm volatile("" : "+v"(ag0), "+v"(ag1), "+v"(ag2));
                        }
                        const float xyz[3] = { rc.x, rc.y, rc.z };
                        const float m = inb_mask(p, xyz);
                        float *dst = out + (b * p.N + o) * 3;
                        if (c == 0) { dst[0] = ag0 * m; dst[1] = ag1 * m; dst[2] = ag2 * m; }
                        else { dst[0] += ag0 * m; dst[1] += ag1 * m; dst[2] += ag2 * m; }
                        continue;
                    }
                    f2 a = { 0.f, 0.f };
#pragma unroll
                    for (int ii = 0; ii <= KSV<K>; ++ii) {
                        if (p.dbg & 2) { a = f2{ w[0].x + wx[ii], w[1].y }; break; }
                        if (K == KMIX && ii > p.order[0]) continue;
                        f2 t2[16];
                        gather_reads(addr + (unsigned)(ii * GPLANE * 8), t2);
                        if constexpr (K == KMIX) clear_unused_taps(p.order[1], p.order[2], t2);
                        f2 pp = { 0.f, 0.f };
#pragma unroll
                        for (int jy = 0; jy <= KSV<K>; ++jy) {
                            f2 q = { 0.f, 0.f };
#pragma unroll
                            for (int k = 0; k <= KSV<K>; ++k) q = f2{ w[k].y, w[k].y } * t2[4 * jy + k] + q;
                            pp = f2{ w[jy].x, w[jy].x } * q + pp;
                        }
                        a = f2{ wx[ii], wx[ii] } * pp + a;
                    }
                    const float xyz[3] = { rc.x, rc.y, rc.z };
                    const float m = inb_mask(p, xyz);
                    const int64_t o = (int64_t)__float_as_int(rc.w);
                    if ((p.dbg & 4) && a.x != 12345.f) continue;
                    oc0[o] = a.x * m;
                    if (two) oc0[p.val_sc + o] = a.y * m;
                }
            }
        }
    }
}

constexpr int NPROBE = 128;
constexpr int BOXVOL = 14500;
constexpr int DENSEVOL = 13000;
constexpr int PULLOUT = 15;
struct ProbeHdr { int gate, done, nslow, nfar, nvalid, nbox, nfull, ncorner; };

template <int K, int GM>
__global__ __launch_bounds__(NT1) void own_probe(KParams p, BrickGrid bg, const float *__restrict__ grid, ProbeHdr *__restrict__ hdr,
                                                 int gx, int gy, int gz, int nty, int ntz, int ntiles, int nbatch, int nch)
{
    __shared__ int lo[3], hi[3], cnt[3], clo[3], chi[3];
    const int tid = threadIdx.x;
    const int64_t total = (int64_t)ntiles * nbatch;
    const int64_t work = (int64_t)blockIdx.x * total / gridDim.x;
    const int64_t b = work / ntiles;
    const TileGeom g = tile_geom((int)(work % ntiles), gx, gy, gz, nty, ntz);
    if (tid < 3) { lo[tid] = 0x7fffffff; hi[tid] = -0x7fffffff; cnt[tid] = 0; clo[tid] = 0x7fffffff; chi[tid] = -0x7fffffff; }
    float fl[VPT1][3];
    unsigned valid = 0, corner = 0;
    int far = 0;
#pragma unroll
    for (int v = 0; v < VPT1; ++v) {
        int ox, oy, oz; float c[3];
        sample_pos(g, tid + NT1 * v, ox, oy, oz);
        if (ox < gx && oy < gy && oz < gz) valid |= 1u << v;
        if (((ox - g.ox0) % (TS - 1)) == 0 && ((oy - g.oy0) % (TS - 1)) == 0 && ((oz - g.oz0) % (TS - 1)) == 0) corner |= 1u << v;
        ox = ox < gx ? ox : gx - 1; oy = oy < gy ? oy : gy - 1; oz = oz < gz ? oz : gz - 1;
        load_xyz<GM>(p, grid, b, g, ox, oy, oz, c);
        bool in = true;
#pragma unroll
        for (int d = 0; d < 3; ++d) {
            fl[v][d] = floorf(c[d] - 0.5f * (float)(K - 1));
            in = in && fl[v][d] >= (float)(bg.lo[d] - OFF) && fl[v][d] < (float)(bg.top[d] + NHI * BR);
            fl[v][d] = __builtin_fmaxf(__builtin_fminf(fl[v][d], 1073741824.f), -1073741824.f);
        }
        if (((valid >> v) & 1) && !in) ++far;
    }
    __syncthreads();
    int mn[3] = { 0x7fffffff, 0x7fffffff, 0x7fffffff }, mx[3] = { -0x7fffffff, -0x7fffffff, -0x7fffffff };
#pragma unroll
    for (int v = 0; v < VPT1; ++v) {
        if (!((valid >> v) & 1)) continue;
#pragma unroll
        for (int d = 0; d < 3; ++d) {
            const int i = fl[v][d] == fl[v][d] ? __float2int_rz(fl[v][d]) : 0;
            mn[d] = i < mn[d] ? i : mn[d]; mx[d] = i > mx[d] ? i : mx[d];
            if ((corner >> v) & 1) { atomicMin(&clo[d], i); atomicMax(&chi[d], i); }
        }
    }
#pragma unroll
    for (int d = 0; d < 3; ++d) {
        const int a = wave_min(mn[d]), e = wave_max(mx[d]);
        if ((tid & 63) == 0) { atomicMin(&lo[d], a); atomicMax(&hi[d], e); }
    }
    __syncthreads();
    const int cap[3] = { 33, 33, 32 };
    int l[3], h[3], boxvol = 1, cornervol = 1;
#pragma unroll
    for (int d = 0; d < 3; ++d) {
        int a = lo[d], sz = hi[d] + K - a + 1;
        if (sz > cap[d]) { a += (sz - cap[d]) / 2; sz = cap[d]; }
        l[d] = a; h[d] = a + sz - K - 1;
        boxvol *= sz > 0 ? sz : 0;
        const int cs = chi[d] + K - clo[d] + 1;
        cornervol *= cs > 0 ? (cs < cap[d] ? cs : cap[d]) : 0;
    }
    int slow = 0, nv = 0;
#pragma unroll
    for (int v = 0; v < VPT1; ++v) {
        if (!((valid >> v) & 1)) continue;
        ++nv;
        bool in = true;
#pragma unroll
        for (int d = 0; d < 3; ++d) {
            const int i = fl[v][d] == fl[v][d] ? __float2int_rz(fl[v][d]) : 0x7fffffff;
            in = in && i >= l[d] && i <= h[d];
        }
        if (!in) ++slow;
    }
    slow = wave_sum(slow); far = wave_sum(far); nv = wave_sum(nv);
    if ((tid & 63) == 0) { atomicAdd(&cnt[0], slow); atomicAdd(&cnt[1], far); atomicAdd(&cnt[2], nv); }
    __syncthreads();
    if (tid == 0) {
        atomicAdd(&hdr->nslow, cnt[0]); atomicAdd(&hdr->nfar, cnt[1]); atomicAdd(&hdr->nvalid, cnt[2]);
        if (cnt[2] == NS) { atomicAdd(&hdr->nbox, boxvol); atomicAdd(&hdr->nfull, 1); atomicAdd(&hdr->ncorner, cornervol); }
        __threadfence();
        if (atomicAdd(&hdr->done, 1) == (int)gridDim.x - 1) {
            const int ns = atomicAdd(&hdr->nslow, 0), nf = atomicAdd(&hdr->nfar, 0), nn = atomicAdd(&hdr->nvalid, 0);
            const int nb = atomicAdd(&hdr->nbox, 0), nt = atomicAdd(&hdr->nfull, 0), nc = atomicAdd(&hdr->ncorner, 0);
            const bool rough = nch > 1 && (int64_t)nb > (int64_t)BOXVOL * nt && (int64_t)nb * 10 > (int64_t)nc * 16;
            const bool dense = (int64_t)nc <= (int64_t)DENSEVOL * nt;
            if (nch == -2) hdr->gate = ((int64_t)ns * 1000 > (int64_t)nn * PULLOUT && (int64_t)nf * 64 <= nn) ? 1 : 0;
            else if (nch < 0) hdr->gate = (((int64_t)ns * 250 > nn || dense) && (int64_t)nf * 64 <= nn) ? 1 : 0;
            else hdr->gate = (((int64_t)ns * 250 > nn || rough) && (int64_t)nf * 64 <= nn) ? 1 : 0;
        }
    }
}

struct Workspace {
    int *flags;
    ProbeHdr *hdr; int *ndesc; int *bmax; uint2 *desc; float4 *rec; float *vals; unsigned short *meta;
    int64_t nrec; int nbricks;
};
static int64_t align256(int64_t x) { return (x + 255) & ~(int64_t)255; }

static int64_t layout(const KParams &k, int B, int ntiles, int nch, void *base, Workspace *w, int64_t nflags = 0, bool shared = false)
{
    const BrickGrid bg = brick_grid(k);
    const int64_t nbricks = (int64_t)bg.per_item * (shared ? 1 : B);
    const int64_t nrec = (int64_t)ntiles * NS * B;
    int64_t o = 0;
    unsigned char *p = (unsigned char *)base;
    const int64_t o_hdr = o; o += 256;
    const int64_t o_nd = o; o += nbricks * 4;
    const int64_t o_bm = o; o += nbricks * 8;
    const int64_t o_fl = o; o += nflags * 4; o = align256(o);
    const int64_t o_desc = o; o += align256(nbricks * (shared ? CAPX : CAPD) * 8);
    const int64_t o_rec = o; o += align256(nrec * 16);
    const int64_t o_val = o; o += align256(nrec * 4 * (nch > 1 ? nch - 1 : 0));
    const int64_t o_meta = o; o += align256(nrec * 2);
    if (w) {
        w->hdr = (ProbeHdr *)(p + o_hdr); w->ndesc = (int *)(p + o_nd); w->desc = (uint2 *)(p + o_desc);
        w->rec = (float4 *)(p + o_rec); w->vals = (float *)(p + o_val); w->meta = (unsigned short *)(p + o_meta);
        w->bmax = (int *)(p + o_bm); w->flags = (int *)(p + o_fl);
        w->nrec = nrec; w->nbricks = (int)nbricks;
    }
    return o;
}

static int tile_count(const interpol_problem *p)
{
    int64_t n = 1;
    for (int d = 0; d < 3; ++d) n *= (p->grid_shape[d] + TS - 1) / TS;
    return n > 0x7fffffff ? 0 : (int)n;
}

int mix_launch_bin(int dtype, int idx, const KParams &k, const BrickGrid &bg, const Workspace &w, const void *val, const void *grid, void *vol,
                   const int *gate, const void *aux, const int *all, int gx, int gy, int gz, int ntiles, int b0, int nb, hipStream_t st, int thin);
int mix_launch_acc(const KParams &k, const BrickGrid &bg, const Workspace &w, void *vol, int nch, int color, int b0, int nb, const int *gate,
                   int *ctr, unsigned nblocks, hipStream_t st);
int mix_launch_gather(int grad, const KParams &k, const BrickGrid &bg, const Workspace &w, const void *vol, void *val, const int *gate,
                      const void *gout, unsigned nblocks, hipStream_t st);

#ifdef IP_OWNER_MIX_TU
int mix_launch_bin(int dtype, int idx, const KParams &k, const BrickGrid &bg, const Workspace &w, const void *val, const void *grid, void *vol,
                   const int *gate, const void *aux, const int *all, int gx, int gy, int gz, int ntiles, int b0, int nb, hipStream_t st, int thin)
{
    const int nty = (gy + TS - 1) / TS, ntz = (gz + TS - 1) / TS;
    const dim3 tgrid((unsigned)(ntiles * nb));
#define IP_MIX_BIN(T, IDX)                                                                                              \
    {                                                                                                                   \
        const int attr = big_lds<own_bin<T, KMIX, 0, IDX>>(sizeof(BinSmem));                                            \
        if (attr) return attr;                                                                                          \
        hipLaunchKernelGGL((own_bin<T, KMIX, 0, IDX>), tgrid, dim3(NT1), sizeof(BinSmem), st, k, bg, (const T *)val, (const float *)grid, \
                           (float *)vol, w.ndesc, w.desc, w.rec, w.vals, w.meta, w.bmax, w.nrec, gx, gy, gz, nty, ntz, ntiles, gate, (const T *)aux, all, ntiles * b0, thin); \
    }
    if (idx == 0) { if (dtype == INTERPOL_F32) IP_MIX_BIN(float, 0) else if (dtype == INTERPOL_BF16) IP_MIX_BIN(bf16_t, 0) else if (dtype == INTERPOL_F16) IP_MIX_BIN(f16_t, 0) else return INTERPOL_E_DTYPE; }
    else if (idx == 1) IP_MIX_BIN(float, 1) else if (idx == 2) IP_MIX_BIN(float, 2) else IP_MIX_BIN(float, 3)
#undef IP_MIX_BIN
    const hipError_t e = hipGetLastError();
    return e == hipSuccess ? 0 : (int)e;
}
int mix_launch_acc(const KParams &k, const BrickGrid &bg, const Workspace &w, void *vol, int nch, int color, int b0, int nb, const int *gate,
                   int *ctr, unsigned nblocks, hipStream_t st)
{
    const int attr = big_lds<own_accumulate<KMIX>>(sizeof(AccSmem));
    if (attr) return attr;
    hipLaunchKernelGGL((own_accumulate<KMIX>), dim3(nblocks), dim3(NT), sizeof(AccSmem), st, k, bg, (const int *)w.ndesc,
                       (const uint2 *)w.desc, (const float4 *)w.rec, (const float *)w.vals, (const unsigned short *)w.meta,
                       (const int *)w.bmax, w.nrec, (float *)vol, nch, color, nb, gate, ctr, b0, (const int *)w.hdr + HDR_SHELL);
    const hipError_t e = hipGetLastError();
    return e == hipSuccess ? 0 : (int)e;
}
int mix_launch_gather(int grad, const KParams &k, const BrickGrid &bg, const Workspace &w, const void *vol, void *val, const int *gate,
                      const void *gout, unsigned nblocks, hipStream_t st)
{
#define IP_MIX_GAT(GR)                                                                                                  \
    {                                                                                                                   \
        const int attr = big_lds<own_gather<KMIX, GR>>(sizeof(GatSmem));                                                \
        if (attr) return attr;                                                                                          \
        hipLaunchKernelGGL((own_gather<KMIX, GR>), dim3(nblocks), dim3(NT), sizeof(GatSmem), st, k, bg, (const int *)w.ndesc, (const uint2 *)w.desc, \
                           (const float4 *)w.rec, (const int *)w.bmax, (int *)w.hdr + 40, (const float *)vol, (float *)val, gate, (const float *)gout); \
    }
    if (grad == 1) IP_MIX_GAT(1) else if (grad == 2) IP_MIX_GAT(2) else IP_MIX_GAT(0)
#undef IP_MIX_GAT
    const hipError_t e = hipGetLastError();
    return e == hipSuccess ? 0 : (int)e;
}
#endif

}

#ifndef IP_OWNER_MIX_TU

static bool shared_target(const interpol_problem *p) { return p->vol_stride[0] == 0 && p->batch > 1; }
static bool mixed_orders(const KParams &k) { return k.order[0] != k.order[1] || k.order[0] != k.order[2]; }
static bool owner_eligible(const interpol_problem *p, const KParams &k, bool scatter = false)
{
    const bool shared = scatter && shared_target(p);
    if (p->dim != 3 || p->batch > 4096) return false;
    if (!(p->flags & (INTERPOL_FLAG_BINNED_SCATTER | INTERPOL_FLAG_AUTO_SCATTER))) return false;
    if (k.order[0] != k.order[1] || k.order[0] != k.order[2]) {
        for (int d = 0; d < 3; ++d) if (k.order[d] < 1 || k.order[d] > 3) return false;
        if (k.sep != 0) return false;
    } else if (k.order[0] < (scatter ? 1 : 2) || k.order[0] > 3) return false;
    int64_t n = 1, nv = 1, nb = shared ? 1 : p->batch;
    for (int d = 0; d < 3; ++d) {
        n *= p->grid_shape[d]; nv *= p->vol_shape[d];
        nb *= owner::NLO + owner::NHI + (p->vol_shape[d] + 15 + owner::BR - 1) / owner::BR;
        if (p->grid_shape[d] > 0x7fffffff / 4) return false;
    }
    const int64_t nt = owner::tile_count(p);
    if (n < 4096 || nt == 0 || nt * owner::NS * p->batch > 0x7fffffffll || nb > 0x7fffffffll / (shared ? owner::CAPX : owner::CAPD)) return false;
    if ((uint64_t)n * 12ull > 0xffffffffull) return false;
    return (shared ? 8 * n * p->batch : 4 * n) >= nv;
}

constexpr int NEAREST_THR16 = 24;
static bool nearest_scatter(const KParams &k) { return k.dim == 3 && k.mode == MODE_ISO0 && k.order[0] == 0 && k.order[1] == 0 && k.order[2] == 0; }
static KParams nearest_as_trilinear(const KParams &k)
{
    KParams q = k;
    if (nearest_scatter(k)) { q.order[0] = 1; q.order[1] = 1; q.order[2] = 1; }
    return q;
}

int64_t owner_workspace_bytes(const interpol_problem *p, const KParams &k_in, bool count_only)
{
    const KParams k = nearest_as_trilinear(k_in);
    if (!owner_eligible(p, k, true)) return 0;
    const int nch = count_only ? 1 : k.C + (k.cc ? 1 : 0);
    return owner::layout(k, (int)p->batch, owner::tile_count(p), nch, nullptr, nullptr, 0, shared_target(p));
}

namespace owner {
template <typename T, int IDX = 0>
static int launch_bin(const interpol_problem *p, const KParams &k, const BrickGrid &bg, const Workspace &w, const void *val, const void *grid,
                      void *vol, const int *gate, hipStream_t st, const void *aux = nullptr, const int *all = nullptr,
                      int b0 = 0, int nb = -1, int thin = 0)
{
    if (nb < 0) nb = (int)p->batch;
    const int gx = (int)p->grid_shape[0], gy = (int)p->grid_shape[1], gz = (int)p->grid_shape[2];
    const int nty = (gy + TS - 1) / TS, ntz = (gz + TS - 1) / TS;
    const int ntiles = tile_count(p);
    const dim3 tgrid((unsigned)(ntiles * nb));
    if (k.order[0] != k.order[1] || k.order[0] != k.order[2])
        return mix_launch_bin(std::is_same<T, float>::value ? INTERPOL_F32 : (std::is_same<T, bf16_t>::value ? INTERPOL_BF16 : INTERPOL_F16), IDX, k, bg, w,
                              val, grid, vol, gate, aux, all, gx, gy, gz, ntiles, b0, nb, st, thin);
#define IP_OWN_BIN(KK, GM)                                                                                              \
    {                                                                                                                   \
        const int attr = big_lds<own_bin<T, KK, GM, IDX>>(sizeof(BinSmem));                                               \
        if (attr) return attr;                                                                                          \
        hipLaunchKernelGGL((own_bin<T, KK, GM, IDX>), tgrid, dim3(NT1), sizeof(BinSmem), st, k, bg, (const T *)val, (const float *)grid, \
                           (float *)vol, w.ndesc, w.desc, w.rec, w.vals, w.meta, w.bmax, w.nrec, gx, gy, gz, nty, ntz, ntiles, gate, (const T *)aux, all, ntiles * b0, thin); \
    }
#define IP_OWN_BY_GM(KK)                                                                                                \
    { if (k.sep == 0) IP_OWN_BIN(KK, 0) else if (k.sep == 1) IP_OWN_BIN(KK, 1) else if (k.sep == 2) IP_OWN_BIN(KK, 2) else IP_OWN_BIN(KK, 3) }
    if (k.order[0] == 3) IP_OWN_BY_GM(3) else if (k.order[0] == 2) IP_OWN_BY_GM(2) else IP_OWN_BY_GM(1)
#undef IP_OWN_BY_GM
#undef IP_OWN_BIN
    return 0;
}
}

static int chain_counter(int chain, int color)
{
    static const int base[CHAIN_SIDE + 1] = { 16, 8 };
    return color < 8 ? base[chain] + color : 24;
}

Route try_owner_push(const interpol_problem *p, const KParams &k_in, const void *val, const void *grid, void *vol,
                     void *workspace, int64_t workspace_bytes, hipStream_t st, const int **gate_out, PendingZero *zf)
{
    using namespace owner;
    const bool nearest = nearest_scatter(k_in);
    const KParams k = nearest_as_trilinear(k_in);
    if (!workspace || !owner_eligible(p, k, true)) return Route::declined();
    const bool count_only = val == nullptr;
    const int nch = count_only ? 1 : k.C + (k.cc ? 1 : 0);
    const int dtype = count_only ? INTERPOL_F32 : p->dtype;
    if (dtype != INTERPOL_F32 && dtype != INTERPOL_BF16 && dtype != INTERPOL_F16) return Route::declined();
    Workspace w;
    if (((uintptr_t)workspace & 255u) != 0) return Route::declined();
    const bool shared = shared_target(p);
    if (layout(k, (int)p->batch, tile_count(p), nch, workspace, &w, 0, shared) > workspace_bytes) return Route::declined();
    BrickGrid bg = brick_grid(k);
    if (shared) { bg.item = 0; bg.capd = CAPX; }
    const bool gated = !(p->flags & INTERPOL_FLAG_BINNED_SCATTER);
    if (nearest && gated && k.sep != 0 && k.sep != 2) return Route::declined();
    const int B = (int)p->batch;
    ChainSet *cs = nullptr;
    if (!shared && B >= 2 && !(p->flags & INTERPOL_FLAG_SERIAL_ITEMS)) {
        hipStreamCaptureStatus cap = hipStreamCaptureStatusNone;
        if (hipStreamIsCapturing(st, &cap) != hipSuccess) { (void)hipGetLastError(); cap = hipStreamCaptureStatusActive; }
        if (cap == hipStreamCaptureStatusNone) cs = chains_acquire();
    }
    bool zero_pending = zf && zf->pending;
    const size_t slice = (size_t)k.vol_sb * 4;
    if (zero_pending && !(cs && zf->ptr == vol && slice * (size_t)B == zf->bytes)) {
        const hipError_t ez = zero_async(zf->ptr, zf->bytes, st);
        if (ez != hipSuccess) { chains_release(cs); return Route::error((int)ez); }
        zf->pending = zero_pending = false;
    }
    hipLaunchKernelGGL(own_zero, dim3((unsigned)((64 + 3ll * w.nbricks + 1023) / 1024)), dim3(1024), 0, st, (int *)w.hdr, 64 + 3 * w.nbricks);
    hipError_t e = hipGetLastError();
    if (e != hipSuccess) { chains_release(cs); return Route::error((int)e); }
    const int *gate = nullptr;
    if (gated && nearest) {
        const int rp = linear_pull_probe(p, k, grid, w.hdr, st, &gate, NEAREST_THR16);
        if (rp) { chains_release(cs); return Route::error(rp); }
    } else if (gated) {
        const int gx = (int)p->grid_shape[0], gy = (int)p->grid_shape[1], gz = (int)p->grid_shape[2];
        const int nty = (gy + TS - 1) / TS, ntz = (gz + TS - 1) / TS, ntiles = tile_count(p);
        const long long total = (long long)ntiles * B;
        const dim3 pgrid((unsigned)(total < NPROBE ? total : NPROBE));
#define IP_OWN_PROBE(KK, GM) hipLaunchKernelGGL((own_probe<KK, GM>), pgrid, dim3(NT1), 0, st, k, bg, (const float *)grid, w.hdr, gx, gy, gz, nty, ntz, ntiles, B, nch);
#define IP_OWN_PROBE_GM(KK) { if (k.sep == 0) IP_OWN_PROBE(KK, 0) else if (k.sep == 1) IP_OWN_PROBE(KK, 1) else if (k.sep == 2) IP_OWN_PROBE(KK, 2) else IP_OWN_PROBE(KK, 3) }
        if (k.order[0] == 3 || mixed_orders(k)) IP_OWN_PROBE_GM(3) else if (k.order[0] == 2) IP_OWN_PROBE_GM(2) else IP_OWN_PROBE_GM(1)
#undef IP_OWN_PROBE_GM
#undef IP_OWN_PROBE
        gate = &w.hdr->gate;
    }
    const int nchain = B < CHAIN_SIDE + 1 ? B : CHAIN_SIDE + 1;
    if (cs) {
        bool ok = hipEventRecord(cs->fork, st) == hipSuccess;
        for (int i = 0; i + 1 < nchain && ok; ++i) ok = hipStreamWaitEvent(cs->side[i], cs->fork, 0) == hipSuccess;
        if (!ok) { (void)hipGetLastError(); chains_release(cs); cs = nullptr; }
    }
    if (zero_pending && !cs) {
        const hipError_t ez = zero_async(zf->ptr, zf->bytes, st);
        if (ez != hipSuccess) return Route::error((int)ez);
        zf->pending = zero_pending = false;
    }
    const long long want = 2ll * cu_count();
    const bool general = (p->flags & INTERPOL_FLAG_GENERAL_KERNELS) != 0;
    static const int thins[4] = { THIN_SHELL_RUN, 4, 64, 16 };
    const int thin = (p->flags & INTERPOL_FLAG_SHELL_RUNS) ? 0 : ((k.dbg & 256) ? -1 : 1) * thins[(k.dbg >> 6) & 3];
    auto enqueue = [&](hipStream_t s, int chain, int b0, int nb) -> int {
        if (zero_pending) {
            const hipError_t ez = zero_async((char *)vol + (size_t)b0 * slice, (size_t)nb * slice, s);
            if (ez != hipSuccess) return (int)ez;
        }
        const int nbin = shared ? B : nb;
        int rc;
        switch (dtype) {
        case INTERPOL_F32: rc = launch_bin<float>(p, k, bg, w, val, grid, vol, gate, s, nullptr, nullptr, b0, nbin, thin); break;
        case INTERPOL_BF16: rc = launch_bin<bf16_t>(p, k, bg, w, val, grid, vol, gate, s, nullptr, nullptr, b0, nbin, thin); break;
        default: rc = launch_bin<f16_t>(p, k, bg, w, val, grid, vol, gate, s, nullptr, nullptr, b0, nbin, thin); break;
        }
        if (rc) return rc;
        for (int color = 0; color < 9; ++color) {
            long long nwork = nb;
            for (int d = 0; d < 3; ++d) nwork *= color_count(color, d, bg);
            if (nwork <= 0) continue;
            const dim3 agrid((unsigned)(nwork < want ? nwork : want));
            int *ctr = (int *)w.hdr + chain_counter(chain, color);
#define IP_OWN_ACC_SH(KK, SH)                                                                                           \
            {                                                                                                           \
                const int attr = big_lds<own_accumulate<KK, false, SH>>(sizeof(AccSmem));                               \
                if (attr) return attr;                                                                                  \
                hipLaunchKernelGGL((own_accumulate<KK, false, SH>), agrid, dim3(NT), sizeof(AccSmem), s, k, bg, (const int *)w.ndesc, \
                                   (const uint2 *)w.desc, (const float4 *)w.rec, (const float *)w.vals, (const unsigned short *)w.meta,  \
                                   (const int *)w.bmax, w.nrec, (float *)vol, nch, color, nb, gate, ctr, b0,           \
                                   (const int *)w.hdr + HDR_SHELL);                                                     \
            }
#define IP_OWN_ACC(KK) { if (color < 8 && !general) IP_OWN_ACC_SH(KK, false) else IP_OWN_ACC_SH(KK, true) }
            if (mixed_orders(k)) { const int rm = mix_launch_acc(k, bg, w, vol, nch, color, b0, nb, gate, ctr, agrid.x, s); if (rm) return rm; }
            else if (k.order[0] == 3) IP_OWN_ACC(3) else if (k.order[0] == 2) IP_OWN_ACC(2)
            else if (nearest) {
                const int attr = big_lds<own_accumulate<1, true>>(sizeof(AccSmem));
                if (attr) return attr;
                hipLaunchKernelGGL((own_accumulate<1, true>), agrid, dim3(NT), sizeof(AccSmem), s, k, bg, (const int *)w.ndesc,
                                   (const uint2 *)w.desc, (const float4 *)w.rec, (const float *)w.vals, (const unsigned short *)w.meta,
                                   (const int *)w.bmax, w.nrec, (float *)vol, nch, color, nb, gate, ctr, b0, (const int *)w.hdr + HDR_SHELL);
            }
            else IP_OWN_ACC(1)
#undef IP_OWN_ACC
#undef IP_OWN_ACC_SH
        }
        const hipError_t el = hipGetLastError();
        return el == hipSuccess ? 0 : (int)el;
    };
    int rc = 0;
    if (!cs) rc = enqueue(st, 0, 0, shared ? 1 : B);
    else {
        for (int c = 1; c <= nchain && rc == 0; ++c) {
            const int ch = c % nchain, b0 = (int)((long long)ch * B / nchain), b1 = (int)((long long)(ch + 1) * B / nchain);
            rc = enqueue(ch ? cs->side[ch - 1] : st, ch, b0, b1 - b0);
        }
        if (zero_pending && rc == 0) zf->pending = false;
        for (int i = 0; i + 1 < nchain; ++i) {
            if (hipEventRecord(cs->join[i], cs->side[i]) == hipSuccess && hipStreamWaitEvent(st, cs->join[i], 0) == hipSuccess) continue;
            (void)hipGetLastError();
            const hipError_t es = hipStreamSynchronize(cs->side[i]);
            if (es != hipSuccess && rc == 0) rc = (int)es;
        }
        chains_release(cs);
    }
    IP_TRY(rc);
    if (gate_out) *gate_out = gate;
    return gated ? Route::gated() : Route::done();
}

static bool owner_pull_eligible(const interpol_problem *p, const KParams &k)
{
    if (p->dtype != INTERPOL_F32 || p->grid_dtype != INTERPOL_F32) return false;
    if (p->val_stride[0] < 0) return false;
    return owner_eligible(p, k);
}
int64_t owner_pull_workspace_bytes(const interpol_problem *p, const KParams &k)
{
    if (!owner_pull_eligible(p, k)) return 0;
    const int nt = owner::tile_count(p);
    return owner::layout(k, (int)p->batch, nt, 1, nullptr, nullptr, (int64_t)nt * p->batch);
}
Route owner_pull_prepare(const interpol_problem *p, const KParams &k, void *workspace, int64_t workspace_bytes, hipStream_t st, int **flags_out, int *nzero_out)
{
    using namespace owner;
    if (!workspace || !owner_pull_eligible(p, k)) return Route::declined();
    if (((uintptr_t)workspace & 255u) != 0) return Route::declined();
    const int nt = tile_count(p);
    const int64_t nflags = (int64_t)nt * p->batch;
    Workspace w;
    if (layout(k, (int)p->batch, nt, 1, workspace, &w, nflags) > workspace_bytes) return Route::declined();
    const int64_t nz = 64 + 3ll * w.nbricks;
    if (nz + nflags > 0x7fffffffll || (int *)w.hdr + nz != w.flags) return Route::declined();
    if (p->flags & INTERPOL_FLAG_BINNED_SCATTER) {
        hipLaunchKernelGGL(own_zero, dim3((unsigned)((nz + 1023) / 1024)), dim3(1024), 0, st, (int *)w.hdr, (int)nz);
        IP_TRY((int)hipGetLastError());
    }
    *flags_out = w.flags;
    *nzero_out = (int)nz;
    return Route::done();
}
int owner_grad_probe(const interpol_problem *p, const KParams &k, const void *grid, void *workspace, int64_t workspace_bytes, hipStream_t st, int mode)
{
    using namespace owner;
    const int ntiles = tile_count(p);
    Workspace w;
    if (layout(k, (int)p->batch, ntiles, 1, workspace, &w, (int64_t)ntiles * p->batch) > workspace_bytes) return INTERPOL_E_SCRATCH;
    const BrickGrid bg = brick_grid(k);
    const int64_t nz = 64 + 3ll * w.nbricks;
    hipLaunchKernelGGL(own_zero, dim3((unsigned)((nz + 1023) / 1024)), dim3(1024), 0, st, (int *)w.hdr, (int)nz);
    const int B = (int)p->batch;
    const int gx = (int)p->grid_shape[0], gy = (int)p->grid_shape[1], gz = (int)p->grid_shape[2];
    const int nty = (gy + TS - 1) / TS, ntz = (gz + TS - 1) / TS;
    const long long total = (long long)ntiles * B;
    const dim3 pgrid((unsigned)(total < NPROBE ? total : NPROBE));
#define IP_OWN_PROBE(KK, GM) hipLaunchKernelGGL((own_probe<KK, GM>), pgrid, dim3(NT1), 0, st, k, bg, (const float *)grid, w.hdr, gx, gy, gz, nty, ntz, ntiles, B, mode);
#define IP_OWN_PROBE_GM(KK) { if (k.sep == 0) IP_OWN_PROBE(KK, 0) else if (k.sep == 1) IP_OWN_PROBE(KK, 1) else if (k.sep == 2) IP_OWN_PROBE(KK, 2) else IP_OWN_PROBE(KK, 3) }
    if (k.order[0] == 3 || mixed_orders(k)) IP_OWN_PROBE_GM(3) else IP_OWN_PROBE_GM(2)
#undef IP_OWN_PROBE_GM
#undef IP_OWN_PROBE
    const hipError_t e = hipGetLastError();
    return e == hipSuccess ? 0 : (int)e;
}
namespace owner {
template <int GM>
__global__ __launch_bounds__(256) void lin_probe(KParams p, const float *__restrict__ grid, int *__restrict__ hdr, int gx, int gy, int gz, int nty, int ntz,
                                                 int ntiles, long long total, int stride, int thr16)
{
    __shared__ int acc[2];
    const int tid = threadIdx.x;
    if (tid < 2) acc[tid] = 0;
    __syncthreads();
    const long long work = (long long)blockIdx.x * stride;
    const long long wk = work < total ? work : total - 1;
    const int64_t b = wk / ntiles;
    const TileGeom g = tile_geom((int)(wk % ntiles), gx, gy, gz, nty, ntz);
    float s = 0.f; int n = 0;
    for (int id = tid; id < TS * TS * TS; id += 512) {
        int ox, oy, oz;
        sample_pos(g, id, ox, oy, oz);
        if (ox >= gx || oy >= gy || oz + 2 >= gz || (id & 15) + 2 >= TS) continue;
        float q0[3], q1[3], q2[3];
        load_xyz<GM>(p, grid, b, g, ox, oy, oz, q0);
        load_xyz<GM>(p, grid, b, g, ox, oy, oz + 1, q1);
        load_xyz<GM>(p, grid, b, g, ox, oy, oz + 2, q2);
        for (int d = 0; d < 3; ++d) s += __builtin_fabsf(q0[d] - 2.f * q1[d] + q2[d]);
        ++n;
    }
    s = s < 1e4f ? s : 1e4f;
    if (n) { atomicAdd(&acc[0], (int)(s * 16.f)); atomicAdd(&acc[1], n); }
    __syncthreads();
    if (tid == 0) {
        const unsigned long long a0 = (unsigned long long)(acc[0] < (1 << 20) ? acc[0] : (1 << 20)), a1 = (unsigned long long)acc[1];
        const unsigned long long add = work < total ? (a0 << 34) | (a1 << 12) | 1ull : 1ull;
        const unsigned long long tot = __hip_atomic_fetch_add(reinterpret_cast<unsigned long long *>(hdr + 2), add, __ATOMIC_RELAXED, __HIP_MEMORY_SCOPE_AGENT) + add;
        if ((tot & 0xfffull) == (unsigned long long)gridDim.x) {
            const unsigned long long sum16 = tot >> 34, cnt = (tot >> 12) & 0x3fffffull;
            __hip_atomic_store(&hdr[0], (cnt > 0 && sum16 > cnt * (unsigned long long)thr16) ? 1 : 0, __ATOMIC_RELAXED, __HIP_MEMORY_SCOPE_AGENT);
        }
    }
}

}

int linear_pull_probe(const interpol_problem *p, const KParams &k, const void *grid, void *workspace, hipStream_t st, const int **gate_out, int thr16)
{
    using namespace owner;
    int *hdr = (int *)workspace;
    hipLaunchKernelGGL(own_zero, dim3(1), dim3(64), 0, st, hdr, 8);
    const int gx = (int)p->grid_shape[0], gy = (int)p->grid_shape[1], gz = (int)p->grid_shape[2];
    const int ntx = (gx + TS - 1) / TS, nty = (gy + TS - 1) / TS, ntz = (gz + TS - 1) / TS, ntiles = ntx * nty * ntz;
    const long long total = (long long)ntiles * p->batch;
    int stride = (int)((total + 511) / 512);
    stride = stride < 1 ? 1 : (stride | 1);
    const unsigned nb = (unsigned)((total + stride - 1) / stride);
    if (k.sep == 0) hipLaunchKernelGGL((lin_probe<0>), dim3(nb), dim3(256), 0, st, k, (const float *)grid, hdr, gx, gy, gz, nty, ntz, ntiles, total, stride, thr16);
    else hipLaunchKernelGGL((lin_probe<2>), dim3(nb), dim3(256), 0, st, k, (const float *)grid, hdr, gx, gy, gz, nty, ntz, ntiles, total, stride, thr16);
    *gate_out = hdr;
    const hipError_t e = hipGetLastError();
    return e == hipSuccess ? 0 : (int)e;
}

int owner_pull_finish(const interpol_problem *p, const KParams &k, const void *vol, const void *grid, void *val,
                      void *workspace, int64_t workspace_bytes, bool all, hipStream_t st, bool grad, const void *gout, bool probed, bool spatial)
{
    using namespace owner;
    const int nt = tile_count(p);
    Workspace w;
    if (layout(k, (int)p->batch, nt, 1, workspace, &w, (int64_t)nt * p->batch) > workspace_bytes) return INTERPOL_E_SCRATCH;
    const BrickGrid bg = brick_grid(k);
    KParams kk = k;
    kk.gate = Gate::none(); kk.tile_flags = nullptr;
    int rc = grad ? launch_bin<float, 2>(p, kk, bg, w, vol, grid, val, all ? nullptr : w.flags, st, gout, probed ? &w.hdr->gate : nullptr)
           : spatial ? launch_bin<float, 3>(p, kk, bg, w, vol, grid, val, nullptr, st, nullptr, probed ? &w.hdr->gate : nullptr)
                  : launch_bin<float, 1>(p, kk, bg, w, vol, grid, val, all ? nullptr : w.flags, st, nullptr, probed ? &w.hdr->gate : nullptr);
    if (rc) return rc;
    const long long want = 2ll * cu_count();
    const dim3 ggrid((unsigned)(w.nbricks < want ? w.nbricks : want));
#define IP_OWN_GAT(KK, GR)                                                                                              \
    {                                                                                                                   \
        const int attr = big_lds<own_gather<KK, GR>>(sizeof(GatSmem));                                                  \
        if (attr) return attr;                                                                                          \
        hipLaunchKernelGGL((own_gather<KK, GR>), ggrid, dim3(NT), sizeof(GatSmem), st, kk, bg, (const int *)w.ndesc, (const uint2 *)w.desc, \
                           (const float4 *)w.rec, (const int *)w.bmax, (int *)w.hdr + 40, (const float *)vol, (float *)val,            \
                           (spatial && probed) ? (const int *)&w.hdr->gate : (const int *)nullptr, (const float *)gout);  \
    }
    if (mixed_orders(k)) {
        const int rm = mix_launch_gather(grad ? 1 : (spatial ? 2 : 0), kk, bg, w, vol, val, (spatial && probed) ? (const int *)&w.hdr->gate : (const int *)nullptr, gout, ggrid.x, st);
        if (rm) return rm;
    }
    else if (grad) { if (k.order[0] == 3) IP_OWN_GAT(3, 1) else IP_OWN_GAT(2, 1) }
    else if (spatial) { if (k.order[0] == 3) IP_OWN_GAT(3, 2) else IP_OWN_GAT(2, 2) }
    else { if (k.order[0] == 3) IP_OWN_GAT(3, 0) else IP_OWN_GAT(2, 0) }
#undef IP_OWN_GAT
    const hipError_t e = hipGetLastError();
    return e == hipSuccess ? 0 : (int)e;
}

}

#ifdef IP_PROF
extern "C" __attribute__((visibility("default"))) int interpol_debug_prof_owner(unsigned long long *out, int reset)
{
    unsigned long long z[16] = { 0 };
    if (out && hipMemcpyFromSymbol(out, HIP_SYMBOL(ip::sorted::g_prof), sizeof z) != hipSuccess) return -1;
    if (reset && hipMemcpyToSymbol(HIP_SYMBOL(ip::sorted::g_prof), z, sizeof z) != hipSuccess) return -1;
    return 0;
}
#endif
#else
}
#endif
#undef IP_KS
#undef IP_KD
#undef IP_WX
#undef IP_MU
#undef IP_RECORD_CELL
```

### torch-interpol_amd/interpol/_hip.py

```python
import ctypes
import threading
import os

import torch

from .sepgrid import SeparableGrid, AffineGrid, LazyGrid

_PKG_ROOT = os.path.dirname(os.path.dirname(os.path.abspath(__file__)))
LIB_PATH = os.environ.get("INTERPOL_HIP_LIB") or os.path.join(_PKG_ROOT, "lib", "libinterpol_hip.so")

ABI_VERSION = 1
F32, F64, BF16, F16 = 0, 1, 2, 3
FLAG_NO_FASTPATH = 1
FLAG_ACCUMULATE = 2
FLAG_FORCE_TILED = 4
FLAG_SEPARABLE_GRID = 8
FLAG_DISPLACEMENT = 16
FLAG_WITH_COUNT = 32
FLAG_BINNED_SCATTER = 64
FLAG_AUTO_SCATTER = 1 << 24
_ROUTED_2D = (torch.float32, torch.bfloat16, torch.float16)
FLAG_SMALL_TILES = 1 << 25
FLAG_SERIAL_ITEMS = 1 << 26
FLAG_GENERAL_KERNELS = 1 << 27
FLAG_SHELL_RUNS = 1 << 28
_POISON_SCRATCH = os.environ.get("INTERPOL_POISON_SCRATCH", "0") not in ("", "0")
_WS_NOCACHE = os.environ.get("INTERPOL_WS_NOCACHE", "0") not in ("", "0")
FLAG_AFFINE_GRID = 128

def _empty(*size, **kw):
    return torch.empty(*size, **kw)


def _scratch(t):
    if _POISON_SCRATCH and t is not None:
        t.view(torch.uint8).fill_(0xff)
    return t


_DTYPE_CODE = {torch.float32: F32, torch.float64: F64, torch.bfloat16: BF16, torch.float16: F16}

SYMBOLS = (
    "interpol_pull", "interpol_push", "interpol_count", "interpol_grad", "interpol_pushgrad",
    "interpol_hess", "interpol_pull_backward", "interpol_push_backward", "interpol_count_backward",
    "interpol_spline_filter", "interpol_spline_filter_to", "interpol_resample_1d", "interpol_resample_1d_gathers", "interpol_pull_labels",
    "interpol_push_bricks", "interpol_push_bricks_workspace", "interpol_host_bound_index", "interpol_host_bound_sign",
    "interpol_host_weight", "interpol_host_weight_f32", "interpol_abi_version",
    "interpol_error_string", "interpol_kernel_name", "interpol_scatter_workspace",
    "interpol_set_handback", "interpol_release_stream", "interpol_has_experiments", "interpol_pull_workspace", "interpol_pull_ws", "interpol_push_backward_ws", "interpol_grad_ws",
    "interpol_affine_backward_workspace", "interpol_pull_backward_affine", "interpol_push_backward_affine",
    "interpol_compose", "interpol_compose_backward_right",
    "interpol_jacobian", "interpol_jacdet_backward_field",
    "interpol_regulariser", "interpol_regulariser_energy_workspace", "interpol_regulariser_energy",
    "interpol_regulariser_solve_workspace", "interpol_regulariser_solve",
    "interpol_ssd_workspace", "interpol_ssd",
    "interpol_ssd_affine_workspace", "interpol_ssd_affine",
    "interpol_mi_affine_workspace", "interpol_mi_affine",
    "interpol_lcc_workspace", "interpol_lcc",
)


class Problem(ctypes.Structure):
    _fields_ = [
        ("abi_version", ctypes.c_int32),
        ("dim", ctypes.c_int32),
        ("dtype", ctypes.c_int32),
        ("grid_dtype", ctypes.c_int32),
        ("extrapolate", ctypes.c_int32),
        ("bound", ctypes.c_int32 * 3),
        ("order", ctypes.c_int32 * 3),
        ("flags", ctypes.c_int32),
        ("batch", ctypes.c_int64),
        ("channels", ctypes.c_int64),
        ("vol_shape", ctypes.c_int64 * 3),
        ("grid_shape", ctypes.c_int64 * 3),
        ("vol_stride", ctypes.c_int64 * 5),
        ("grid_stride", ctypes.c_int64 * 5),
        ("val_stride", ctypes.c_int64 * 7),
    ]


_lib = None


class HipExtensionMissing(ImportError):
    pass


_WS_CACHE = {}
_WS_MAX = 4
_WS_DENIED = {}
_WS_CHECK_ABOVE = 64 << 20


def release_workspaces():
    _WS_CACHE.clear()
    _WS_DENIED.clear()


def _available(idx):
    free, _ = torch.cuda.mem_get_info(idx)
    return free + torch.cuda.memory_reserved(idx) - torch.cuda.memory_allocated(idx)


def _optional_workspace(nbytes, dev):
    if nbytes <= 0:
        return None
    idx = dev.index if dev.index is not None else torch.cuda.current_device()
    if torch.cuda.is_current_stream_capturing() or _WS_NOCACHE:
        try:
            return _empty(nbytes, dtype=torch.uint8, device=dev)
        except torch.cuda.OutOfMemoryError:
            return None
    key = (idx, int(torch.cuda.current_stream(dev).cuda_stream), threading.get_ident())
    ws = _WS_CACHE.get(key)
    if ws is not None and ws.numel() >= nbytes:
        _WS_CACHE[key] = _WS_CACHE.pop(key)
        return ws
    avail = None
    if nbytes > _WS_CHECK_ABOVE:
        if ws is not None:
            del _WS_CACHE[key]
            ws = None
        avail = _available(idx)
        denied = _WS_DENIED.get(idx)
        if denied is not None and nbytes >= denied[0] and avail < denied[1] + denied[0] // 2:
            return None
        if 2 * nbytes > avail:
            return None
    try:
        ws = _empty(nbytes, dtype=torch.uint8, device=dev)
    except torch.cuda.OutOfMemoryError:
        _WS_DENIED[idx] = (nbytes, avail if avail is not None else _available(idx))
        return None
    if _WS_DENIED:
        _WS_DENIED.pop(idx, None)
    _WS_CACHE.pop(key, None)
    _WS_CACHE[key] = ws
    while len(_WS_CACHE) > _WS_MAX:
        _WS_CACHE.pop(next(iter(_WS_CACHE)))
    return ws


def lib():
    global _lib
    if _lib is not None:
        return _lib
    if not os.path.exists(LIB_PATH):
        raise HipExtensionMissing(
            "libinterpol_hip.so not found at %s: build it with `make -C %s -j8` "
            "(or `python -c 'import __graft_entry__ as g; g.build()'`). "
            "There is no CPU fallback." % (LIB_PATH, _PKG_ROOT))
    L = ctypes.CDLL(LIB_PATH)
    vp, i64, i32 = ctypes.c_void_p, ctypes.c_int64, ctypes.c_int32
    pp = ctypes.POINTER(Problem)
    L.interpol_pull.argtypes = [pp, vp, vp, vp, vp]
    L.interpol_grad.argtypes = [pp, vp, vp, vp, vp]
    L.interpol_hess.argtypes = [pp, vp, vp, vp, vp]
    L.interpol_push.argtypes = [pp, vp, vp, vp, vp, i64, vp]
    L.interpol_pushgrad.argtypes = [pp, vp, vp, vp, vp, i64, vp]
    L.interpol_count.argtypes = [pp, vp, vp, vp, i64, vp]
    L.interpol_pull_backward.argtypes = [pp, vp, vp, vp, vp, vp, vp, i64, vp]
    L.interpol_push_backward.argtypes = [pp, vp, vp, vp, vp, vp, vp]
    L.interpol_count_backward.argtypes = [pp, vp, vp, vp, vp]
    L.interpol_spline_filter.argtypes = [vp, i32, i64, i64, i64, i32, i32, vp]
    L.interpol_spline_filter_to.argtypes = [vp, vp, i32, i64, i64, i64, i32, i32, vp]
    L.interpol_pull_labels.argtypes = [pp, vp, vp, vp, vp]
    L.interpol_push_bricks.argtypes = [pp, vp, vp, vp, vp, i64, vp]
    L.interpol_push_bricks.restype = ctypes.c_int
    L.interpol_push_bricks_workspace.argtypes = [pp]
    L.interpol_push_bricks_workspace.restype = i64
    L.interpol_scatter_workspace.argtypes = [pp, i32]
    L.interpol_scatter_workspace.restype = i64
    L.interpol_pull_workspace.argtypes = [pp]
    L.interpol_pull_workspace.restype = i64
    L.interpol_pull_ws.argtypes = [pp, vp, vp, vp, vp, i64, vp]
    L.interpol_pull_ws.restype = ctypes.c_int
    L.interpol_grad_ws.argtypes = [pp, vp, vp, vp, vp, i64, vp]
    L.interpol_grad_ws.restype = ctypes.c_int
    L.interpol_push_backward_ws.argtypes = [pp, vp, vp, vp, vp, vp, vp, i64, vp]
    L.interpol_push_backward_ws.restype = ctypes.c_int
    L.interpol_affine_backward_workspace.argtypes = [pp]
    L.interpol_affine_backward_workspace.restype = i64
    L.interpol_pull_backward_affine.argtypes = [pp, vp, vp, vp, vp, vp, i64, vp]
    L.interpol_pull_backward_affine.restype = ctypes.c_int
    L.interpol_push_backward_affine.argtypes = [pp, vp, vp, vp, vp, vp, i64, vp]
    L.interpol_push_backward_affine.restype = ctypes.c_int
    L.interpol_compose.argtypes = [pp, vp, vp, vp, vp]
    L.interpol_compose.restype = ctypes.c_int
    L.interpol_compose_backward_right.argtypes = [pp, vp, vp, vp, vp, vp]
    L.interpol_compose_backward_right.restype = ctypes.c_int
    L.interpol_jacobian.argtypes = [pp, vp, vp, i32, i32, vp]
    L.interpol_jacobian.restype = ctypes.c_int
    L.interpol_jacdet_backward_field.argtypes = [pp, vp, vp, vp, vp]
    L.interpol_jacdet_backward_field.restype = ctypes.c_int
    f64, dp = ctypes.c_double, ctypes.POINTER(ctypes.c_double)
    L.interpol_regulariser.argtypes = [pp, vp, vp, f64, f64, f64, dp, vp]
    L.interpol_regulariser.restype = ctypes.c_int
    L.interpol_regulariser_energy_workspace.argtypes = [pp]
    L.interpol_regulariser_energy_workspace.restype = i64
    L.interpol_regulariser_energy.argtypes = [pp, vp, vp, f64, f64, f64, dp, vp, i64, vp]
    L.interpol_regulariser_energy.restype = ctypes.c_int
    L.interpol_regulariser_solve_workspace.argtypes = [pp, i32]
    L.interpol_regulariser_solve_workspace.restype = i64
    L.interpol_regulariser_solve.argtypes = [pp, vp, vp, i32, i64, vp, f64, f64, f64, dp, i32, f64, vp, vp, i64, vp]
    L.interpol_regulariser_solve.restype = ctypes.c_int
    L.interpol_ssd_workspace.argtypes = [pp]
    L.interpol_ssd_workspace.restype = i64
    L.interpol_ssd.argtypes = [pp, vp, vp, vp, vp, vp, vp, vp, i32, i64, i64, i64, vp, i64, vp]
    L.interpol_ssd.restype = ctypes.c_int
    L.interpol_ssd_affine_workspace.argtypes = [pp]
    L.interpol_ssd_affine_workspace.restype = i64
    L.interpol_ssd_affine.argtypes = [pp, vp, vp, vp, vp, vp, vp, vp, i32, i64, i64, vp, i64, vp]
    L.interpol_ssd_affine.restype = ctypes.c_int
    L.interpol_mi_affine_workspace.argtypes = [pp, i32]
    L.interpol_mi_affine_workspace.restype = i64
    L.interpol_mi_affine.argtypes = [pp, vp, vp, vp, vp, vp, vp, vp, vp, vp, i32, i32, i64, i64, vp, i64, vp]
    L.interpol_mi_affine.restype = ctypes.c_int
    L.interpol_lcc_workspace.argtypes = [pp]
    L.interpol_lcc_workspace.restype = i64
    L.interpol_lcc.argtypes = [pp, vp, vp, vp, vp, vp, vp, vp, i32, ctypes.POINTER(ctypes.c_int), ctypes.c_double, i64, i64, i64, vp, i64, vp]
    L.interpol_lcc.restype = ctypes.c_int
    L.interpol_set_handback.argtypes = [i32]
    L.interpol_set_handback.restype = i32
    L.interpol_release_stream.argtypes = [ctypes.c_void_p]
    L.interpol_release_stream.restype = i32
    L.interpol_resample_1d.argtypes = [i32, i32, i32, i32, i32, i32, i32, i64, i64, i64, i64, vp, vp, vp, vp]
    L.interpol_resample_1d_gathers.argtypes = [i32, i64, i64]
    L.interpol_resample_1d_gathers.restype = i32
    for name in ("interpol_pull", "interpol_grad", "interpol_hess", "interpol_push", "interpol_pushgrad",
                 "interpol_count", "interpol_pull_backward", "interpol_push_backward",
                 "interpol_count_backward", "interpol_spline_filter", "interpol_spline_filter_to", "interpol_resample_1d", "interpol_pull_labels"):
        getattr(L, name).restype = ctypes.c_int
    L.interpol_host_bound_index.argtypes = [i32, i32, i32]
    L.interpol_host_bound_index.restype = i32
    L.interpol_host_bound_sign.argtypes = [i32, i32, i32]
    L.interpol_host_bound_sign.restype = i32
    L.interpol_host_weight.argtypes = [i32, ctypes.c_double, i32]
    L.interpol_host_weight.restype = ctypes.c_double
    L.interpol_host_weight_f32.argtypes = [i32, ctypes.c_float, i32]
    L.interpol_host_weight_f32.restype = ctypes.c_float
    L.interpol_abi_version.restype = i32
    L.interpol_error_string.argtypes = [ctypes.c_int]
    L.interpol_error_string.restype = ctypes.c_char_p
    L.interpol_kernel_name.argtypes = [pp, ctypes.c_char_p]
    L.interpol_kernel_name.restype = ctypes.c_char_p
    if L.interpol_abi_version() != ABI_VERSION:
        raise HipExtensionMissing("libinterpol_hip.so has ABI version %d, expected %d: rebuild it"
                                  % (L.interpol_abi_version(), ABI_VERSION))
    _lib = L
    return L


def _check(rc, what):
    if rc == 0:
        return
    msg = lib().interpol_error_string(rc).decode()
    if rc == -2:
        raise NotImplementedError("%s: %s" % (what, msg))
    if rc == -8:
        raise NotImplementedError("%s: %s" % (what, msg))
    if rc in (-1, -3, -5, -7):
        raise ValueError("%s: %s" % (what, msg))
    raise RuntimeError("%s failed: %s (code %d)" % (what, msg, rc))


def _require_gpu(*tensors):
    dev = None
    for t in tensors:
        if t is None:
            continue
        if not t.is_cuda:
            raise RuntimeError(
                "interpol (MI355X build): tensors must live on a ROCm GPU; got a %s tensor. "
                "This build has no CPU path." % t.device.type)
        if dev is None:
            dev = t.device
        elif t.device != dev:
            raise RuntimeError("interpol: all tensors must be on the same device (%s vs %s)" % (dev, t.device))
    return dev


def _stream(dev):
    return ctypes.c_void_p(torch.cuda.current_stream(dev).cuda_stream)


def _ptr(t):
    return ctypes.c_void_p(t.data_ptr()) if t is not None else ctypes.c_void_p(0)


def common_dtypes(img, grid):
    if not grid.dtype.is_floating_point:
        raise TypeError("grid must be a floating point tensor")
    idt = img.dtype if img is not None else grid.dtype
    if not idt.is_floating_point:
        raise TypeError("image must be a floating point tensor")
    if idt == torch.float64 or grid.dtype == torch.float64:
        return torch.float64, torch.float64
    if idt in (torch.bfloat16, torch.float16):
        return idt, torch.float32
    return torch.float32, torch.float32


def _spatially_contiguous(t, first_spatial):
    expect = 1
    for d in range(t.dim() - 1, first_spatial - 1, -1):
        if t.shape[d] > 1 and t.stride(d) != expect:
            return False
        expect *= t.shape[d]
    return True


def _bstride(t, B):
    return 0 if (t.shape[0] == 1 and B > 1) else t.stride(0)


def make_problem(dim, dtype, grid_dtype, bound, order, extrapolate, B, C, vol_shape, grid_shape,
                 vol_stride, grid_stride, val_stride, flags=0):
    p = Problem()
    p.abi_version = ABI_VERSION
    p.dim = dim
    p.dtype = _DTYPE_CODE[dtype]
    p.grid_dtype = _DTYPE_CODE[grid_dtype]
    p.extrapolate = int(extrapolate)
    for d in range(3):
        p.bound[d] = int(bound[d]) if d < dim else 1
        p.order[d] = int(order[d]) if d < dim else 0
        p.vol_shape[d] = int(vol_shape[d]) if d < dim else 1
# ... 1039 lines not shown
```

Measured before the change: 33700.

## Skip volume read-back in owner accumulate for bricks not yet written

Adds a per-brick dirty map that the direct and orphan scatter paths set whenever they touch a brick. When the output still has a pending zero-fill, the colour accumulate pass uses this map to find untouched bricks, computes the region each brick owns alone, and stores there without first loading the old volume values. The aim is to cut global read traffic in the read-modify-write flush. In exchange it adds dirty-marking work in the scatter paths, enlarges the zeroed header, and brings in a new RMW_FLUSH flag that turns the path off.

```diff
diff --git a/include/interpol_hip.h b/include/interpol_hip.h
--- a/include/interpol_hip.h
+++ b/include/interpol_hip.h
@@ -61,6 +61,7 @@
 #define INTERPOL_FLAG_SERIAL_ITEMS (1 << 26)
 #define INTERPOL_FLAG_GENERAL_KERNELS (1 << 27)
 #define INTERPOL_FLAG_SHELL_RUNS (1 << 28)
+#define INTERPOL_FLAG_RMW_FLUSH (1 << 29)
 #define INTERPOL_FLAG_AFFINE_GRID   128
 
 int64_t interpol_scatter_workspace(const interpol_problem *p, int32_t count_only);
diff --git a/torch-interpol_amd/csrc/owner_geom.hpp b/torch-interpol_amd/csrc/owner_geom.hpp
--- /dev/null
+++ b/torch-interpol_amd/csrc/owner_geom.hpp
@@ -0,0 +1,84 @@
+#pragma once
+
+#ifdef __HIPCC__
+#define IP_GEOM_HD __host__ __device__ __forceinline__
+#else
+#define IP_GEOM_HD inline
+#endif
+
+namespace ip {
+namespace owner {
+
+constexpr int BR = 16;
+constexpr int OFF = 160;
+constexpr int BOX = BR + 3;
+
+constexpr int NLO = OFF / BR, NHI = (OFF + 3 + BR - 1) / BR;
+struct BrickGrid {
+    int nb[3];
+    int lo[3], top[3], nin[3], split[3];
+    int per_item;
+    int item;
+    int capd;
+};
+IP_GEOM_HD void brick_grid_dim(BrickGrid &g, int d, int K, int n, bool f)
+{
+    g.lo[d] = f ? -(BOX - 1) / 2 : 0;
+    g.top[d] = f ? n - (BOX + 1) / 2 + BR : (n - K > 0 ? n - K : 0);
+    g.nin[d] = (g.top[d] - g.lo[d] + BR - 1) / BR;
+    if (f) {
+        const int c = g.top[d] - g.lo[d] - BR * (g.nin[d] - 1);
+        if (c < K) { g.top[d] -= c; g.nin[d] -= 1; }
+    }
+    g.split[d] = f ? g.nin[d] / 2 : (g.nin[d] > 0 ? g.nin[d] - 1 : 0);
+    g.nb[d] = NLO + g.nin[d] + NHI;
+}
+IP_GEOM_HD int brick_and_cell(int ft, int lo, int top, int nin, int split)
+{
+    if (ft < lo) return ((ft - lo + OFF) >> 4) | (((ft - lo + OFF) & (BR - 1)) << 16);
+    if (ft >= top) return (NLO + nin + ((ft - top) >> 4)) | (((ft - top) & (BR - 1)) << 16);
+    const int u = ft - lo, v = top - 1 - ft;
+    const bool hi = u >= BR * split && (v >> 4) < nin - 1 - split;
+    return hi ? (NLO + nin - 1 - (v >> 4)) | ((BR - 1 - (v & (BR - 1))) << 16) : (NLO + (u >> 4)) | ((u & (BR - 1)) << 16);
+}
+IP_GEOM_HD int brick_origin(int bk, int lo, int top, int nin, int split)
+{
+    if (bk < NLO) return lo + bk * BR - OFF;
+    if (bk >= NLO + nin) return top + (bk - NLO - nin) * BR;
+    const int j = bk - NLO;
+    return j <= split ? lo + j * BR : top - (nin - j) * BR;
+}
+
+IP_GEOM_HD int color_first(int color, int d)
+{
+    if (color >= 8) return 0;
+    const int par = (color >> (2 - d)) & 1;
+    return NLO + ((par - NLO) & 1);
+}
+IP_GEOM_HD int color_bit(int bk) { return bk & 1; }
+
+IP_GEOM_HD void fresh_range(int bk, int d, const BrickGrid &g, int &f_lo, int &f_hi)
+{
+    f_lo = 0; f_hi = BOX;
+    const int j = bk - NLO;
+    if (j < 0 || j >= g.nin[d] || !color_bit(bk)) return;
+    const int o = brick_origin(bk, g.lo[d], g.top[d], g.nin[d], g.split[d]);
+    if (j > 0) f_lo = brick_origin(bk - 1, g.lo[d], g.top[d], g.nin[d], g.split[d]) + BOX - o;
+    if (j + 1 < g.nin[d]) f_hi = brick_origin(bk + 1, g.lo[d], g.top[d], g.nin[d], g.split[d]) - o;
+    f_lo = f_lo < 0 ? 0 : (f_lo > BOX ? BOX : f_lo);
+    f_hi = f_hi < 0 ? 0 : (f_hi > BOX ? BOX : f_hi);
+}
+
+IP_GEOM_HD void bricks_over(int x, int d, const BrickGrid &g, int &k_lo, int &k_hi)
+{
+    k_lo = 0; k_hi = -1;
+    if (g.nin[d] <= 0 || x < g.lo[d]) return;
+    const int cell = x < g.top[d] ? x : g.top[d] - 1;
+    k_hi = brick_and_cell(cell, g.lo[d], g.top[d], g.nin[d], g.split[d]) & 0xffff;
+    if (brick_origin(k_hi, g.lo[d], g.top[d], g.nin[d], g.split[d]) + BOX <= x) { k_hi = -1; return; }
+    k_lo = k_hi;
+    while (k_lo > NLO && brick_origin(k_lo - 1, g.lo[d], g.top[d], g.nin[d], g.split[d]) + BOX > x) --k_lo;
+}
+
+}
+}
diff --git a/torch-interpol_amd/csrc/push_owner.hip b/torch-interpol_amd/csrc/push_owner.hip
--- a/torch-interpol_amd/csrc/push_owner.hip
+++ b/torch-interpol_amd/csrc/push_owner.hip
@@ -1,14 +1,12 @@
 #include "sorted_util.hpp"
 #include "route.hpp"
+#include "owner_geom.hpp"
 
 namespace ip {
 namespace owner {
 
 using namespace sorted;
 
-constexpr int BR = 16;
-constexpr int OFF = 160;
-constexpr int BOX = BR + 3;
 constexpr int PZ = BOX;
 constexpr int PLANE = BOX * PZ;
 constexpr int BOXSLOTS = BOX * PLANE;
@@ -19,6 +17,7 @@
 constexpr int NS = TS * TS * TS;
 constexpr int NT1 = 512, VPT1 = NS / NT1;
 constexpr int LB = 6, NBIN = LB * LB * LB;
+constexpr int NZERO_PER_BRICK = 4;
 constexpr int HDR_SHELL = 34;
 constexpr int THIN_SHELL_RUN = 16;
 constexpr int KMIX = 13;
@@ -36,52 +35,16 @@
 #define IP_MU magic_units<K>()
 #endif
 
-constexpr int NLO = OFF / BR, NHI = (OFF + 3 + BR - 1) / BR;
-struct BrickGrid {
-    int nb[3];
-    int lo[3], top[3], nin[3], split[3];
-    int per_item;
-    int item;
-    int capd;
-};
 __host__ __device__ __forceinline__ bool folds(int bound, int n) { return (bound == B_REPLICATE || bound == B_DCT1 || bound == B_DCT2) && n >= 2 * BR; }
 static BrickGrid brick_grid(const KParams &k)
 {
     BrickGrid g;
     const bool mixed = k.order[0] != k.order[1] || k.order[0] != k.order[2];
-    for (int d = 0; d < 3; ++d) {
-        const int K = mixed ? 3 : k.order[d], n = k.vol_n[d];
-        const bool f = folds(k.bound[d], n);
-        g.lo[d] = f ? -(BOX - 1) / 2 : 0;
-        g.top[d] = f ? n - (BOX + 1) / 2 + BR : (n - K > 0 ? n - K : 0);
-        g.nin[d] = (g.top[d] - g.lo[d] + BR - 1) / BR;
-        if (f) {
-            const int c = g.top[d] - g.lo[d] - BR * (g.nin[d] - 1);
-            if (c < K) { g.top[d] -= c; g.nin[d] -= 1; }
-        }
-        g.split[d] = f ? g.nin[d] / 2 : (g.nin[d] > 0 ? g.nin[d] - 1 : 0);
-        g.nb[d] = NLO + g.nin[d] + NHI;
-    }
+    for (int d = 0; d < 3; ++d) brick_grid_dim(g, d, mixed ? 3 : k.order[d], k.vol_n[d], folds(k.bound[d], k.vol_n[d]));
     g.per_item = g.nb[0] * g.nb[1] * g.nb[2];
     g.item = g.per_item; g.capd = 128;
     return g;
 }
-__host__ __device__ __forceinline__ int brick_and_cell(int ft, int lo, int top, int nin, int split)
-{
-    if (ft < lo) return ((ft - lo + OFF) >> 4) | (((ft - lo + OFF) & (BR - 1)) << 16);
-    if (ft >= top) return (NLO + nin + ((ft - top) >> 4)) | (((ft - top) & (BR - 1)) << 16);
-    const int u = ft - lo, v = top - 1 - ft;
-    const bool hi = u >= BR * split && (v >> 4) < nin - 1 - split;
-    return hi ? (NLO + nin - 1 - (v >> 4)) | ((BR - 1 - (v & (BR - 1))) << 16) : (NLO + (u >> 4)) | ((u & (BR - 1)) << 16);
-}
-__host__ __device__ __forceinline__ int brick_origin(int bk, int lo, int top, int nin, int split)
-{
-    if (bk < NLO) return lo + bk * BR - OFF;
-    if (bk >= NLO + nin) return top + (bk - NLO - nin) * BR;
-    const int j = bk - NLO;
-    return j <= split ? lo + j * BR : top - (nin - j) * BR;
-}
-
 __device__ __forceinline__ bool shell_brick(const KParams &p, const BrickGrid &bg, int b0, int b1, int b2)
 {
     const int bc[3] = { b0, b1, b2 };
@@ -107,9 +70,56 @@
     return m * Cvt<float, T>::ld(val[b * p.val_sb + ch * p.val_sc + o]);
 }
 
+__device__ __forceinline__ void mark_bricks(const BrickGrid &bg, int *__restrict__ dirty, int64_t b, const int *k_lo, const int *k_hi)
+{
+#pragma unroll 1
+    for (int i = k_lo[0]; i <= k_hi[0]; ++i)
+#pragma unroll 1
+        for (int j = k_lo[1]; j <= k_hi[1]; ++j)
+#pragma unroll 1
+            for (int k = k_lo[2]; k <= k_hi[2]; ++k) dirty[(int)b * bg.item + (i * bg.nb[1] + j) * bg.nb[2] + k] = 1;
+}
+__device__ __forceinline__ void mark_stencil(const Lattice &L, const BrickGrid &bg, int *__restrict__ dirty, int64_t b, int i0, int i1, int i2)
+{
+    int kl[3], kh[3], pl[3] = { 0, 0, 0 }, ph[3] = { -2, -2, -2 };
+#pragma unroll 1
+    for (int i = 0; i <= L.k[0]; ++i) {
+        bricks_over((int)(wrap_outofline(L.bound[0], i0 + i, L.n[0]) & 0xffffffffll), 0, bg, kl[0], kh[0]);
+        if (kl[0] == pl[0] && kh[0] == ph[0]) continue;
+        pl[0] = kl[0]; ph[0] = kh[0]; ph[1] = -2;
+#pragma unroll 1
+        for (int j = 0; j <= L.k[1]; ++j) {
+            bricks_over((int)(wrap_outofline(L.bound[1], i1 + j, L.n[1]) & 0xffffffffll), 1, bg, kl[1], kh[1]);
+            if (kl[1] == pl[1] && kh[1] == ph[1]) continue;
+            pl[1] = kl[1]; ph[1] = kh[1]; ph[2] = -2;
+#pragma unroll 1
+            for (int k = 0; k <= L.k[2]; ++k) {
+                bricks_over((int)(wrap_outofline(L.bound[2], i2 + k, L.n[2]) & 0xffffffffll), 2, bg, kl[2], kh[2]);
+                if (kl[2] == pl[2] && kh[2] == ph[2]) continue;
+                pl[2] = kl[2]; ph[2] = kh[2];
+                mark_bricks(bg, dirty, b, kl, kh);
+            }
+        }
+    }
+}
+__device__ __forceinline__ void mark_tap(const Lattice &L, const BrickGrid &bg, int *__restrict__ dirty, int64_t b, const float *x, int tap)
+{
+    const int k1[3] = { L.k[0] + 1, L.k[1] + 1, L.k[2] + 1 };
+    if (tap >= k1[0] * k1[1] * k1[2]) return;
+    const int tp[3] = { tap / (k1[1] * k1[2]), (tap / k1[2]) % k1[1], tap % k1[2] };
+    int kl[3], kh[3];
+#pragma unroll
+    for (int d = 0; d < 3; ++d) {
+        int i0; float t;
+        split(L.k[d], x[d], i0, t);
+        bricks_over((int)(wrap_outofline(L.bound[d], i0 + tp[d], L.n[d]) & 0xffffffffll), d, bg, kl[d], kh[d]);
+    }
+    mark_bricks(bg, dirty, b, kl, kh);
+}
+
 template <typename T, int K, int GM>
 __device__ __forceinline__ void scatter_direct(const KParams &p, const T *__restrict__ val, const float *__restrict__ grid, float *__restrict__ vol,
-                                            int64_t b, TileGeom g, int tid, unsigned mask, int nch)
+                                            int64_t b, TileGeom g, int tid, unsigned mask, int nch, const BrickGrid &bg, int *__restrict__ dirty)
 {
     Lattice L;
 #pragma unroll
@@ -129,6 +139,10 @@
             const long long pk2 = wrap_outofline(L.bound[2], __float2int_rn(rintf(x[2])), L.n[2]);
             const float sgn = (float)((int)(pk0 >> 32) * (int)(pk1 >> 32) * (int)(pk2 >> 32));
             float *q = vol + b * p.vol_sb + (int)(pk0 & 0xffffffffll) * L.ss[0] + (int)(pk1 & 0xffffffffll) * L.ss[1] + (int)(pk2 & 0xffffffffll) * L.ss[2];
+            int kl[3], kh[3];
+            bricks_over((int)(pk0 & 0xffffffffll), 0, bg, kl[0], kh[0]); bricks_over((int)(pk1 & 0xffffffffll), 1, bg, kl[1], kh[1]);
+            bricks_over((int)(pk2 & 0xffffffffll), 2, bg, kl[2], kh[2]);
+            mark_bricks(bg, dirty, b, kl, kh);
 #pragma unroll 1
             for (int ch = 0; ch < nch; ++ch)
                 __hip_atomic_fetch_add(q + (int64_t)ch * p.vol_sc, src_value<T>(p, val, b, o, ch, m) * sgn, __ATOMIC_RELAXED, __HIP_MEMORY_SCOPE_AGENT);
@@ -137,6 +151,7 @@
         int ii[3]; float tt[3];
 #pragma unroll
         for (int d = 0; d < 3; ++d) split(kd<K>(p, d), x[d], ii[d], tt[d]);
+        mark_stencil(L, bg, dirty, b, ii[0], ii[1], ii[2]);
 #pragma unroll 1
         for (int ch = 0; ch < nch; ++ch)
             tiled::scatter_one_thread(L, vol + b * p.vol_sb + ch * p.vol_sc, src_value<T>(p, val, b, o, ch, m), ii[0], ii[1], ii[2], tt[0], tt[1], tt[2]);
@@ -145,7 +160,7 @@
 
 template <typename T, int K, int GM>
 __device__ __forceinline__ void scatter_orphans(const KParams &p, const T *__restrict__ val, const float *__restrict__ grid, float *__restrict__ vol,
-                                             int64_t b, TileGeom g, int tid, unsigned mask, int nch)
+                                             int64_t b, TileGeom g, int tid, unsigned mask, int nch, const BrickGrid &bg, int *__restrict__ dirty)
 {
     Lattice L;
 #pragma unroll
@@ -166,6 +181,7 @@
             if (KSV<K> == 1 && p.mode == MODE_ISO0) { x[0] = rintf(x[0]); x[1] = rintf(x[1]); x[2] = rintf(x[2]); }
             int off;
             const float w = tiled::tap_weight_t<-1, -1>(L, x[0], x[1], x[2], tid & 63, &off, nullptr);
+            mark_tap(L, bg, dirty, b, x, tid & 63);
             float *q = vol + b * p.vol_sb + off;
 #pragma unroll 1
             for (int ch = 0; ch < nch && w != 0.f; ++ch)
@@ -265,7 +281,7 @@
                                                float4 *__restrict__ rec, float *__restrict__ vals, unsigned short *__restrict__ meta,
                                                int *__restrict__ bmax, int64_t nrec,
                                                int gx, int gy, int gz, int nty, int ntz, int ntiles, const int *__restrict__ gate,
-                                               const T *__restrict__ aux, const int *__restrict__ all, int blk0, int thin)
+                                               const T *__restrict__ aux, const int *__restrict__ all, int blk0, int thin, int *__restrict__ dirty)
 {
     const int blk = (int)blockIdx.x + blk0;
     if (IDX) { const bool every = all && *all == 1; if (gate ? (gate[blk] == 0 && !every) : (all && !every)) return; }
@@ -448,12 +464,12 @@
         for (int v = 0; v < VPT1; ++v)
             if (((local >> v) & 1) && sm.cnt[lbin[v] & 255] < 0) orphan |= 1u << v;
         if (IDX) direct |= orphan;
-        else scatter_orphans<T, K, GM>(p, val, grid, vol, b, g, tid, orphan, nch);
+        else scatter_orphans<T, K, GM>(p, val, grid, vol, b, g, tid, orphan, nch, bg, dirty);
     }
     if (IDX == 3) { if (direct) grad_direct<T, K, GM>(p, val, grid, reinterpret_cast<T *>(vol), b, g, tid, direct); return; }
     if (IDX == 2) { if (direct) gradc_direct<T, K, GM>(p, val, aux, grid, vol, b, g, tid, direct); return; }
     if (IDX) { if (direct) gather_direct<T, K, GM>(p, val, grid, reinterpret_cast<T *>(vol), b, g, tid, direct); return; }
-    if (direct) scatter_direct<T, K, GM>(p, val, grid, vol, b, g, tid, direct, nch);
+    if (direct) scatter_direct<T, K, GM>(p, val, grid, vol, b, g, tid, direct, nch, bg, dirty);
 }
 
 constexpr int VPT = 12;
@@ -656,12 +672,6 @@
     x0 = (__float2int_rz(fx) - b0[0]) & (BR - 1); y0 = (__float2int_rz(fy) - b0[1]) & (BR - 1); z0 = (__float2int_rz(fz) - b0[2]) & (BR - 1);
 }
 
-__host__ __device__ __forceinline__ int color_first(int color, int d)
-{
-    if (color >= 8) return 0;
-    const int par = (color >> (2 - d)) & 1;
-    return NLO + ((par - NLO) & 1);
-}
 __host__ __device__ __forceinline__ int color_count(int color, int d, const BrickGrid &bg)
 {
     if (color >= 8) return bg.nb[d];
@@ -711,11 +721,11 @@
                                                         const float4 *__restrict__ rec, const float *__restrict__ vals,
                                                         const unsigned short *__restrict__ meta, const int *__restrict__ bmax, int64_t nrec,
                                                         float *__restrict__ vol, int nch, int color, int nbatch, const int *__restrict__ gate,
-                                                        int *__restrict__ ctr, int bfirst, const int *__restrict__ shell)
+                                                        int *__restrict__ ctr, int bfirst, const int *__restrict__ aux)
 {
     if (gate && *gate != 1) return;
     static_assert(SHELL || (K != KMIX && !NEAR), "the colour instantiation: isotropic orders 1 - 3");
-    if (SHELL) { if (color == 8 && *shell == 0) return; }
+    if (SHELL) { if (color == 8 && *aux == 0) return; }
     else __builtin_assume(color >= 0 && color < 8);
     extern __shared__ __attribute__((aligned(16))) unsigned char smem_raw[];
     AccSmem &sm = *reinterpret_cast<AccSmem *>(smem_raw);
@@ -822,6 +832,13 @@
             }
             if (tid == 63) { sm.n = incl; sm.npieces = inclp; sm.dmax = 0; sm.cmax[0] = 0; sm.cmax[1] = 0; }
             if (SHELL && tid < 3) { sm.rlo[tid] = BR; sm.rhi[tid] = -1; }
+            if constexpr (!SHELL) {
+                if (tid < 3) {
+                    int f_lo = BOX, f_hi = 0;
+                    if (aux != nullptr && aux[brick] == 0) fresh_range(bxyz[tid], tid, bg, f_lo, f_hi);
+                    sm.rlo[tid] = f_lo; sm.rhi[tid] = f_hi;
+                }
+            }
         } else if (atomic && tid < 64 + 3 * 32) {
             const int d = (tid - 64) >> 5, slot = tid & 31;
             if (slot < BOX) {
@@ -1203,10 +1220,16 @@
             }
             if (fixedpt && !atomic && !wide && !(p.dbg & 1)) {
                 constexpr int UF2 = 7;
+                int fl0 = BOX, fh0 = 0, fl1 = BOX, fh1 = 0, fl2 = BOX, fh2 = 0;
+                if constexpr (!SHELL) {
+                    fl0 = __builtin_amdgcn_readfirstlane(sm.rlo[0]); fh0 = __builtin_amdgcn_readfirstlane(sm.rhi[0]);
+                    fl1 = __builtin_amdgcn_readfirstlane(sm.rlo[1]); fh1 = __builtin_amdgcn_readfirstlane(sm.rhi[1]);
+                    fl2 = __builtin_amdgcn_readfirstlane(sm.rlo[2]); fh2 = __builtin_amdgcn_readfirstlane(sm.rhi[2]);
+                }
 #pragma unroll 1
                 for (int e0 = tid; e0 < BOXSLOTS; e0 += UF2 * NT) {
                     int off[UF2]; float t0[UF2], t1[UF2];
-                    unsigned nz = 0, nst[UF2];
+                    unsigned nz = 0, ld = 0, nst[UF2];
 #pragma unroll
                     for (int u = 0; u < UF2; ++u) {
                         const int e = e0 + u * NT;
@@ -1215,13 +1238,14 @@
                             const int xr = e / PLANE, rem = e - xr * PLANE, yr = rem / PZ, zr = rem - yr * PZ;
                             off[u] = (b0[0] + xr) * L.ss[0] + (b0[1] + yr) * L.ss[1] + (b0[2] + zr) * L.ss[2];
                             nst[u] = stencils_at(sm, xr, yr, zr);
-                            if (nst[u] != 0u) nz |= 1u << u;
+                            const bool fresh = !SHELL && xr >= fl0 && xr < fh0 && yr >= fl1 && yr < fh1 && zr >= fl2 && zr < fh2;
+                            if (nst[u] != 0u) { nz |= 1u << u; if (!fresh) ld |= 1u << u; }
                         }
                     }
 #pragma unroll
                     for (int u = 0; u < UF2; ++u) {
-                        t0[u] = ((nz >> u) & 1) ? vc0[off[u]] : 0.f;
-                        t1[u] = (((nz >> u) & 1) && two) ? vc1[off[u]] : 0.f;
+                        t0[u] = ((ld >> u) & 1) ? vc0[off[u]] : 0.f;
+                        t1[u] = (((ld >> u) & 1) && two) ? vc1[off[u]] : 0.f;
                     }
 #pragma unroll
                     for (int u = 0; u < UF2; ++u) {
@@ -1656,6 +1680,7 @@
 struct Workspace {
     int *flags;
     ProbeHdr *hdr; int *ndesc; int *bmax; uint2 *desc; float4 *rec; float *vals; unsigned short *meta;
+    int *dirty;
     int64_t nrec; int nbricks;
 };
 static int64_t align256(int64_t x) { return (x + 255) & ~(int64_t)255; }
@@ -1670,6 +1695,7 @@
     const int64_t o_hdr = o; o += 256;
     const int64_t o_nd = o; o += nbricks * 4;
     const int64_t o_bm = o; o += nbricks * 8;
+    const int64_t o_dy = o; o += nbricks * 4;
     const int64_t o_fl = o; o += nflags * 4; o = align256(o);
     const int64_t o_desc = o; o += align256(nbricks * (shared ? CAPX : CAPD) * 8);
     const int64_t o_rec = o; o += align256(nrec * 16);
@@ -1678,7 +1704,7 @@
     if (w) {
         w->hdr = (ProbeHdr *)(p + o_hdr); w->ndesc = (int *)(p + o_nd); w->desc = (uint2 *)(p + o_desc);
         w->rec = (float4 *)(p + o_rec); w->vals = (float *)(p + o_val); w->meta = (unsigned short *)(p + o_meta);
-        w->bmax = (int *)(p + o_bm); w->flags = (int *)(p + o_fl);
+        w->bmax = (int *)(p + o_bm); w->dirty = (int *)(p + o_dy); w->flags = (int *)(p + o_fl);
         w->nrec = nrec; w->nbricks = (int)nbricks;
     }
     return o;
@@ -1709,7 +1735,7 @@
         const int attr = big_lds<own_bin<T, KMIX, 0, IDX>>(sizeof(BinSmem));                                            \
         if (attr) return attr;                                                                                          \
         hipLaunchKernelGGL((own_bin<T, KMIX, 0, IDX>), tgrid, dim3(NT1), sizeof(BinSmem), st, k, bg, (const T *)val, (const float *)grid, \
-                           (float *)vol, w.ndesc, w.desc, w.rec, w.vals, w.meta, w.bmax, w.nrec, gx, gy, gz, nty, ntz, ntiles, gate, (const T *)aux, all, ntiles * b0, thin); \
+                           (float *)vol, w.ndesc, w.desc, w.rec, w.vals, w.meta, w.bmax, w.nrec, gx, gy, gz, nty, ntz, ntiles, gate, (const T *)aux, all, ntiles * b0, thin, w.dirty); \
     }
     if (idx == 0) { if (dtype == INTERPOL_F32) IP_MIX_BIN(float, 0) else if (dtype == INTERPOL_BF16) IP_MIX_BIN(bf16_t, 0) else if (dtype == INTERPOL_F16) IP_MIX_BIN(f16_t, 0) else return INTERPOL_E_DTYPE; }
     else if (idx == 1) IP_MIX_BIN(float, 1) else if (idx == 2) IP_MIX_BIN(float, 2) else IP_MIX_BIN(float, 3)
@@ -1808,7 +1834,7 @@
         const int attr = big_lds<own_bin<T, KK, GM, IDX>>(sizeof(BinSmem));                                               \
         if (attr) return attr;                                                                                          \
         hipLaunchKernelGGL((own_bin<T, KK, GM, IDX>), tgrid, dim3(NT1), sizeof(BinSmem), st, k, bg, (const T *)val, (const float *)grid, \
-                           (float *)vol, w.ndesc, w.desc, w.rec, w.vals, w.meta, w.bmax, w.nrec, gx, gy, gz, nty, ntz, ntiles, gate, (const T *)aux, all, ntiles * b0, thin); \
+                           (float *)vol, w.ndesc, w.desc, w.rec, w.vals, w.meta, w.bmax, w.nrec, gx, gy, gz, nty, ntz, ntiles, gate, (const T *)aux, all, ntiles * b0, thin, w.dirty); \
     }
 #define IP_OWN_BY_GM(KK)                                                                                                \
     { if (k.sep == 0) IP_OWN_BIN(KK, 0) else if (k.sep == 1) IP_OWN_BIN(KK, 1) else if (k.sep == 2) IP_OWN_BIN(KK, 2) else IP_OWN_BIN(KK, 3) }
@@ -1852,13 +1878,14 @@
         if (cap == hipStreamCaptureStatusNone) cs = chains_acquire();
     }
     bool zero_pending = zf && zf->pending;
+    const int *first_writer = zero_pending && !shared && !(p->flags & INTERPOL_FLAG_RMW_FLUSH) ? w.dirty : nullptr;
     const size_t slice = (size_t)k.vol_sb * 4;
     if (zero_pending && !(cs && zf->ptr == vol && slice * (size_t)B == zf->bytes)) {
         const hipError_t ez = zero_async(zf->ptr, zf->bytes, st);
         if (ez != hipSuccess) { chains_release(cs); return Route::error((int)ez); }
         zf->pending = zero_pending = false;
     }
-    hipLaunchKernelGGL(own_zero, dim3((unsigned)((64 + 3ll * w.nbricks + 1023) / 1024)), dim3(1024), 0, st, (int *)w.hdr, 64 + 3 * w.nbricks);
+    hipLaunchKernelGGL(own_zero, dim3((unsigned)((64 + (long long)NZERO_PER_BRICK * w.nbricks + 1023) / 1024)), dim3(1024), 0, st, (int *)w.hdr, 64 + NZERO_PER_BRICK * w.nbricks);
     hipError_t e = hipGetLastError();
     if (e != hipSuccess) { chains_release(cs); return Route::error((int)e); }
     const int *gate = nullptr;
@@ -1918,7 +1945,7 @@
                 hipLaunchKernelGGL((own_accumulate<KK, false, SH>), agrid, dim3(NT), sizeof(AccSmem), s, k, bg, (const int *)w.ndesc, \
                                    (const uint2 *)w.desc, (const float4 *)w.rec, (const float *)w.vals, (const unsigned short *)w.meta,  \
                                    (const int *)w.bmax, w.nrec, (float *)vol, nch, color, nb, gate, ctr, b0,           \
-                                   (const int *)w.hdr + HDR_SHELL);                                                     \
+                                   SH ? (const int *)w.hdr + HDR_SHELL : first_writer);                                 \
             }
 #define IP_OWN_ACC(KK) { if (color < 8 && !general) IP_OWN_ACC_SH(KK, false) else IP_OWN_ACC_SH(KK, true) }
             if (mixed_orders(k)) { const int rm = mix_launch_acc(k, bg, w, vol, nch, color, b0, nb, gate, ctr, agrid.x, s); if (rm) return rm; }
@@ -1979,7 +2006,7 @@
     const int64_t nflags = (int64_t)nt * p->batch;
     Workspace w;
     if (layout(k, (int)p->batch, nt, 1, workspace, &w, nflags) > workspace_bytes) return Route::declined();
-    const int64_t nz = 64 + 3ll * w.nbricks;
+    const int64_t nz = 64 + (long long)NZERO_PER_BRICK * w.nbricks;
     if (nz + nflags > 0x7fffffffll || (int *)w.hdr + nz != w.flags) return Route::declined();
     if (p->flags & INTERPOL_FLAG_BINNED_SCATTER) {
         hipLaunchKernelGGL(own_zero, dim3((unsigned)((nz + 1023) / 1024)), dim3(1024), 0, st, (int *)w.hdr, (int)nz);
@@ -1996,7 +2023,7 @@
     Workspace w;
     if (layout(k, (int)p->batch, ntiles, 1, workspace, &w, (int64_t)ntiles * p->batch) > workspace_bytes) return INTERPOL_E_SCRATCH;
     const BrickGrid bg = brick_grid(k);
-    const int64_t nz = 64 + 3ll * w.nbricks;
+    const int64_t nz = 64 + (long long)NZERO_PER_BRICK * w.nbricks;
     hipLaunchKernelGGL(own_zero, dim3((unsigned)((nz + 1023) / 1024)), dim3(1024), 0, st, (int *)w.hdr, (int)nz);
     const int B = (int)p->batch;
     const int gx = (int)p->grid_shape[0], gy = (int)p->grid_shape[1], gz = (int)p->grid_shape[2];
diff --git a/torch-interpol_amd/interpol/_hip.py b/torch-interpol_amd/interpol/_hip.py
--- a/torch-interpol_amd/interpol/_hip.py
+++ b/torch-interpol_amd/interpol/_hip.py
@@ -24,6 +24,7 @@
 FLAG_SERIAL_ITEMS = 1 << 26
 FLAG_GENERAL_KERNELS = 1 << 27
 FLAG_SHELL_RUNS = 1 << 28
+FLAG_RMW_FLUSH = 1 << 29
 _POISON_SCRATCH = os.environ.get("INTERPOL_POISON_SCRATCH", "0") not in ("", "0")
 _WS_NOCACHE = os.environ.get("INTERPOL_WS_NOCACHE", "0") not in ("", "0")
 FLAG_AFFINE_GRID = 128
```

Measured after the change: 34170, median of 6. 1.01x the previous value.
